# actuday6418/ray-tracer-s8

Hardware: AMD Instinct MI355X
Metric: Mrays/sec @ 4K/8spp 1024-sphere (higher is better)
Workload: dtype f32

## Files before the change

### ray_tracer_s8_amd/csrc/rt_api.hip

```cpp
#include <hip/hip_runtime.h>
#include <dlfcn.h>

#include <algorithm>
#include <chrono>
#include <cmath>
#include <cstdarg>
#include <cstdio>
#include <cstdlib>
#include <cstring>
#include <atomic>
#include <climits>
#include <condition_variable>
#include <memory>
#include <mutex>
#include <new>
#include <stdexcept>
#include <string>
#include <thread>
#include <vector>

#include "rt_assign.h"
#include "rt_bvh.h"
#include "rt_device.h"
#include "rt_frame_plan.h"
#include "rt_kernel.hip.h"
#include "rt_plan.h"
#include "rt_query.hip.h"
#include "rt_scene_host.h"
#include "rt_trace.hip.h"
#include "rt_bounce.hip.h"
#include "rt_direct.hip.h"
#include "rt_nee.hip.h"
#include "rt_aov.hip.h"
#include "rt_camera.hip.h"
#include "rt_denoise.hip.h"
#include "rt_tile.h"
#ifdef RT_DEBUG_HOOKS
#include "rt_unit.hip.h"
#endif

namespace {

thread_local std::string g_err;

int fail(int code, const std::string& msg) {
    g_err = msg;
    return code;
}

void set_err_noexcept(const char* what) noexcept {
    try {
        g_err = what;
    } catch (...) {
    }
}
template <class F>
int guarded(F&& body) noexcept {
    try {
        return body();
    } catch (const std::bad_alloc&) {
        set_err_noexcept("host allocation failed");
        return RT_ERR_OOM;
    } catch (const std::exception& e) {
        set_err_noexcept(e.what());
        return RT_ERR_HIP;
    } catch (...) {
        set_err_noexcept("internal error");
        return RT_ERR_HIP;
    }
}

#define HIPCHK(expr)                                                                                  \
    do {                                                                                              \
        hipError_t _e = (expr);                                                                       \
        if (_e != hipSuccess)                                                                         \
            return fail(RT_ERR_HIP, std::string(#expr) + ": " + hipGetErrorString(_e) + " (" __FILE__ \
                                                                                        ":" +         \
                                        std::to_string(__LINE__) + ")");                              \
    } while (0)

using rtdev::DevArray;
using rtdev::Event;
using rtdev::EventPool;
using rtdev::GrowBuf;
using rtdev::Stream;

int reserve(GrowBuf& buf, size_t bytes, const char* what) {
    if (buf.grow(bytes) == hipSuccess) return RT_OK;
    (void)hipGetLastError();
    return fail(RT_ERR_OOM, std::string("hipMalloc(") + what + ") failed");
}

struct DeviceCtx {
    int dev = -1;
    Stream stream;
    Stream copy_stream;
    int n_cu = 0;
    std::mutex mu;
};

enum DebugKnob {
    DBG_LDS_TREE = 0,
    DBG_CULL_WALK,
    DBG_NO_STAGE,
    DBG_SLOTS,
    DBG_FORCE_CAPPED,
    DBG_STACK_LDS,
    DBG_COMPACT,
    DBG_REFILL_EIGHTHS,
    DBG_COMMIT_SLOTS,
    DBG_VERBOSE,
    DBG_REORDER,
    DBG_TAIL_TILES,
    DBG_STRIP_COST,
    DBG_DENOISE_LDS_STEP,
    DBG_N
};
std::atomic<int> g_dbg[DBG_N];
const struct { const char* env; int def; } g_dbg_spec[DBG_N] = {
    {"RT_LDS_TREE", 1}, {"RT_CULL_WALK", -1}, {"RT_NO_STAGE", 0}, {"RT_SLOTS", 0}, {"RT_FORCE_CAPPED", 0},
    {"RT_STACK_LDS", 0}, {"RT_COMPACT", 1}, {"RT_REFILL_EIGHTHS", 0}, {"RT_COMMIT_SLOTS", 0}, {"RT_VERBOSE", 0}, {"RT_REORDER", 1}, {"RT_TAIL_TILES", -1}, {"RT_STRIP_COST", 1},
    {"RT_DENOISE_LDS_STEP", -1}};
std::once_flag g_dbg_once;
void dbg_load_env() {
    std::call_once(g_dbg_once, [] {
        for (int k = 0; k < DBG_N; k++) {
            const char* e = getenv(g_dbg_spec[k].env);
            int v = g_dbg_spec[k].def;
            if (e) v = k == DBG_VERBOSE ? 1 : atoi(e);
            g_dbg[k].store(v, std::memory_order_relaxed);
        }
    });
}
inline int dbg(DebugKnob k) { return g_dbg[k].load(std::memory_order_relaxed); }

std::mutex g_mu;
bool g_init = false;
std::vector<DeviceCtx*> g_ctx;
std::atomic<int> g_live_scenes{0};

rtplan::Knobs plan_knobs() {
    rtplan::Knobs k;
    k.lds_tree = dbg(DBG_LDS_TREE);
    k.cull_walk = dbg(DBG_CULL_WALK);
    k.no_stage = dbg(DBG_NO_STAGE);
    k.slots = dbg(DBG_SLOTS);
    k.commit_slots = dbg(DBG_COMMIT_SLOTS);
    k.force_capped = dbg(DBG_FORCE_CAPPED);
    k.stack_lds = dbg(DBG_STACK_LDS);
    k.compact = dbg(DBG_COMPACT);
    k.refill_eighths = dbg(DBG_REFILL_EIGHTHS);
    k.tail_tiles = dbg(DBG_TAIL_TILES);
    return k;
}

}

struct rt_scene {
    DeviceCtx* ctx = nullptr;
    rtplan::SceneShape shape;
    uint32_t n_lights = 0;
    DevArray<uint32_t> d_lights;
    DevArray<float> d_light_c;
    DevArray<float> d_light_ip;
    float light_total = 0.f;
    std::vector<uint32_t> light_world;
    std::vector<float> light_p;
    rtplan::Pose pose;
    bool has_pose = false;
    uint32_t light_sampling = RT_LIGHTS_AREA;
    uint32_t glossy_sampling = RT_GLOSSY_BOUNCE;
    DevArray<float4> d_geom;
    DevArray<float4> d_geom_pk;
    DevArray<float4> d_geom_px;
    DevArray<float4> d_mat;
    DevArray<float> d_emis;
    DevArray<float> d_tri;
    DevArray<float4> d_tri_box;
    DevArray<float4> d_bvh;
    DevArray<float4> d_trav;
    GrowBuf stack_ovf;
    DevArray<uint4> d_travq;
    DevArray<float4> d_geom_r;
    DevArray<uint32_t> d_big;
    uint32_t n_big = 0;
    float tri_k = 0.f, tri_diag = 0.f, tri_es = 0.f, tri_e = 0.f;
    rtbvh::QGrid grid;
    DevArray<uint32_t> d_leaf_of;
    DevArray<uint32_t> d_world_rank;
    bool has_order = false;
    float bvh_build_ms = 0.f;
    DevArray<unsigned long long> d_counters;
    struct Ring {
        GrowBuf buf;
        hipStream_t last = nullptr;
        uint64_t stamp = 0;
    };
    Ring rings[4];
    uint64_t ring_clock = 0;
    GrowBuf d_out, d_outf, d_acc, d_cost;
    GrowBuf d_stage;
    EventPool events;
    uint64_t primary_rays = 0;
    float h2d_ms = 0.f;
    uint32_t last_engine = 0, last_form = 0;
    std::mutex mu;
};

namespace {

int check_request(const rt_tile_request* rq) {
    if (!rq) return fail(RT_ERR_BAD_ARG, "request is NULL");
    if (rq->width == 0 || rq->height == 0 || rq->divisions == 0 || rq->spp == 0)
        return fail(RT_ERR_BAD_ARG, "width, height, divisions and spp must be non-zero");
    if (rq->division_no >= rq->divisions) return fail(RT_ERR_BAD_ARG, "division_no >= divisions");
    if (rq->height / rq->divisions == 0) return fail(RT_ERR_BAD_ARG, "height / divisions == 0 rows");
    if (rq->max_bounces > RT_MAX_BOUNCES) return fail(RT_ERR_LIMIT, "max_bounces > RT_MAX_BOUNCES");
    if (rq->spp > RT_MAX_SPP) return fail(RT_ERR_LIMIT, "spp > RT_MAX_SPP");
    if (rq->reserved != 0) return fail(RT_ERR_BAD_ARG, "reserved must be 0");
    if ((uint64_t)rq->width * rq->height > 0x7fffffffull) return fail(RT_ERR_LIMIT, "image too large");
    return RT_OK;
}

constexpr uint32_t QUEUE_SLOTS = 16384;
#ifdef RT_PROFILE_TIME
constexpr uint32_t COUNTER_WORDS = 4 + QUEUE_SLOTS + 16 * 8192;
#else
constexpr uint32_t COUNTER_WORDS = 4 + QUEUE_SLOTS;
#endif

int check_slot(const rt_scene* sc) {
    if (sc->events.pending().size() >= QUEUE_SLOTS) return fail(RT_ERR_LIMIT, "too many uncollected launches: call rt_scene_collect()");
    return RT_OK;
}

template <class P>
int enqueue(rt_scene* sc, hipStream_t stream, void (*kern)(const P), uint32_t blocks, uint32_t block, size_t lds, const P& p) {
    EventPool::Lease ev;
    int rc = check_slot(sc);
    if (rc) return rc;
    HIPCHK(sc->events.lease(ev));
    HIPCHK(hipEventRecord(ev.a(), stream));
    hipLaunchKernelGGL(kern, dim3(blocks), dim3(block), lds, stream, p);
    HIPCHK(hipGetLastError());
    HIPCHK(hipEventRecord(ev.b(), stream));
    ev.to_pending();
    return RT_OK;
}

struct Grid {
    uint32_t blocks = 0;
    int per_cu = 0;
};
template <class P>
int persistent_blocks(const rt_scene* sc, void (*kern)(const P), uint32_t block, size_t lds, uint64_t items, Grid& g) {
    HIPCHK(hipOccupancyMaxActiveBlocksPerMultiprocessor(&g.per_cu, kern, (int)block, lds));
    if (g.per_cu < 1) g.per_cu = 1;
    g.blocks = (uint32_t)std::min<uint64_t>((items + block - 1) / block, (uint64_t)sc->ctx->n_cu * (uint32_t)g.per_cu);
    return RT_OK;
}

void scene_refs(const rt_scene* sc, bool full_chain, rtk::SceneRefs& r) {
    r.n_sph = sc->shape.n_sph;
    r.n_tri = sc->shape.n_tri;
    r.root_ref = sc->shape.root_ref;
    r.full_chain = full_chain ? 1u : 0u;
    r.trav = sc->d_trav.get();
    r.bvh_nodes = sc->d_bvh.get();
    r.leaf_of = sc->d_leaf_of.get();
    r.world_rank = sc->has_order ? sc->d_world_rank.get() : nullptr;
    r.geom_r = sc->d_geom_r.get();
    r.tri = sc->d_tri.get();
    r.counters = sc->d_counters.get();
}

struct Pass {
    uint32_t begin, end;
    void* const* d_acc;
};
int acquire_stack_ovf(rt_scene* sc, size_t words) {
    HIPCHK(sc->stack_ovf.grow(words * sizeof(uint32_t)));
    return RT_OK;
}

int acquire_ring(rt_scene* sc, hipStream_t stream, size_t bytes, rt_scene::Ring*& rg) {
    rg = nullptr;
    for (auto& r : sc->rings)
        if (r.buf.data() && r.last == stream) { rg = &r; break; }
    if (!rg)
        for (auto& r : sc->rings)
            if (!r.buf.data()) { rg = &r; break; }
    if (!rg) {
        rg = &sc->rings[0];
        for (auto& r : sc->rings)
            if (r.stamp < rg->stamp) rg = &r;
    }
    HIPCHK(rg->buf.grow(bytes));
    if (!rg->buf.done) HIPCHK(rg->buf.done.create(hipEventDisableTiming));
    else if (rg->last != stream) HIPCHK(hipStreamWaitEvent(stream, rg->buf.done.get(), 0));
    rg->last = stream;
    rg->stamp = ++sc->ring_clock;
    return RT_OK;
}

int launch_batch(rt_scene* sc, const rt_tile_request* rqs, uint32_t n, void* const* d_rgb, void* const* d_f32,
                 hipStream_t stream, unsigned long long* d_strip_cost = nullptr, const Pass* pass = nullptr) {
    const rtplan::Knobs kn = plan_knobs();
    const rtplan::SceneShape& sh = sc->shape;
    rtk::KParams p;
    std::memset(&p, 0, sizeof p);
    const rtplan::SampleRange smp = pass ? rtplan::SampleRange{pass->begin, pass->end, true} : rtplan::SampleRange{0u, rqs[0].spp, false};
    rtplan::Plan pl = rtplan::plan_launch(sh, rqs[0], n, smp, kn, p, sc->has_pose ? &sc->pose : nullptr);
    if (pl.status != RT_OK) return fail(pl.status, pl.error);
    p.geom_pk = sc->d_geom_pk.get();
    p.geom_px = sc->d_geom_px.get();
    p.geom = sc->d_geom.get();
    p.mat = sc->d_mat.get();
    p.emis = sc->d_emis.get();
    p.tri = sc->d_tri.get();
    p.tri_box = sc->d_tri_box.get();
    p.bvh_nodes = sc->d_bvh.get();
    p.trav = sc->d_trav.get();
    p.travq = sc->d_travq.get();
    p.geom_r = sc->d_geom_r.get();
    for (int i = 0; i < 3; i++) {
        p.q_base[i] = sc->grid.base[i];
        p.q_step[i] = sc->grid.step[i];
        p.q_rstep[i] = 1.0f / sc->grid.step[i];
    }
    p.leaf_of = sc->d_leaf_of.get();
    p.world_rank = sc->has_order ? sc->d_world_rank.get() : nullptr;
    p.big = sc->d_big.get();
    p.n_big = sc->n_big;
    p.r_slack = sh.r_slack;
    p.tri_k = sc->tri_k;
    p.tri_diag = sc->tri_diag;
    p.tri_es = sc->tri_es;
    p.tri_e = sc->tri_e;
    for (uint32_t i = 0; i < n; i++) {
        p.strips[i].seed = rqs[i].seed;
        p.strips[i].rgb = (uint8_t*)d_rgb[i];
        p.strips[i].f32 = d_f32 ? (float*)d_f32[i] : nullptr;
        p.strips[i].acc = pass ? (float*)pass->d_acc[i] : nullptr;
        p.strips[i].y0 = p.Hs * rqs[i].division_no;
    }
    int rc = check_slot(sc);
    if (rc) return rc;
    p.counters = sc->d_counters.get();
    p.queue = sc->d_counters.get() + 4 + sc->events.pending().size();
    p.strip_cost = dbg(DBG_STRIP_COST) ? d_strip_cost : nullptr;

    const rtk::KernelFn kern = pl.isect < 2 ? rtk::kernel_linear(pl.isect, pl.expanded) : rtk::kernel_traverse(pl.isect, pl.count_steps);
    int per_cu = 0;
    HIPCHK(hipOccupancyMaxActiveBlocksPerMultiprocessor(&per_cu, kern, pl.block, pl.lds));
    if (per_cu < 1) per_cu = 1;
    if (dbg(DBG_VERBOSE))
        fprintf(stderr, "[rt] engine %d%s  lds %zu B  workgroups/CU %d  leaf slots %u  bvh depth %u  leaf density %.3f  prims %u\n",
                pl.engine, pl.capped ? " (capped stack)" : "", pl.lds, per_cu, pl.maxl_l2, sh.bvh_depth, sh.leaf_density, sh.n_sph + sh.n_tri);
    rtplan::plan_queue(pl, (uint32_t)sc->ctx->n_cu * (uint32_t)per_cu, kn, p);
    p.stack_ovf = nullptr;
    if (pl.capped) {
        if ((rc = acquire_stack_ovf(sc, pl.ovf_words))) return rc;
        p.stack_ovf = (uint32_t*)sc->stack_ovf.data();
    }
    if (dbg(DBG_VERBOSE))
        fprintf(stderr, "[rt] sample-unit ring %zu B: %u units per pixel, %u slots of %u records per wave\n", pl.ring_bytes, p.upp, p.n_slots,
                p.slot_stride);
    rt_scene::Ring* rg = nullptr;
    if ((rc = acquire_ring(sc, stream, pl.ring_bytes, rg))) return rc;
    p.ring = (float*)rg->buf.data();
    if (p.stack_ovf) {
        if (sc->stack_ovf.done) HIPCHK(hipStreamWaitEvent(stream, sc->stack_ovf.done.get(), 0));
        else HIPCHK(sc->stack_ovf.done.create(hipEventDisableTiming));
    }
    HIPCHK(hipMemsetAsync(p.queue, 0, sizeof(unsigned long long), stream));
    sc->last_engine = (uint32_t)pl.engine;
    sc->last_form = pl.expanded ? 1u : 0u;
    if ((rc = enqueue(sc, stream, kern, pl.blocks, pl.block, pl.lds, p))) return rc;
    HIPCHK(hipEventRecord(rg->buf.done.get(), stream));
    if (p.stack_ovf) HIPCHK(hipEventRecord(sc->stack_ovf.done.get(), stream));
    sc->primary_rays += (uint64_t)p.Hs * p.W * p.upp * n;
    return RT_OK;
}

int collect_locked(rt_scene* sc, rt_tile_stats* st) {
    float ms = 0.f;
    uint32_t n = 0;
    for (const EventPool::Pair& pr : sc->events.pending()) {
        HIPCHK(hipEventSynchronize(pr.b));
        float t = 0.f;
        HIPCHK(hipEventElapsedTime(&t, pr.a, pr.b));
        ms += t;
        n++;
    }
    sc->events.collected();
    unsigned long long c[4] = {0, 0, 0, 0};
    HIPCHK(hipMemcpy(c, sc->d_counters.get(), sizeof c, hipMemcpyDeviceToHost));
    HIPCHK(hipMemset(sc->d_counters.get(), 0, sizeof c));
    if (st) {
        st->ray_segments = c[0];
        st->broad_candidates = c[1];
        st->exact_fallbacks = c[2];
        st->primary_rays = sc->primary_rays;
        st->kernel_ms = ms;
        st->n_launches = n;
        st->h2d_ms = sc->h2d_ms;
        st->d2h_ms = 0.f;
        st->engine = sc->last_engine;
        st->broad_form = sc->last_form;
        st->node_steps = c[3];
    }
    sc->primary_rays = 0;
    sc->h2d_ms = 0.f;
    return RT_OK;
}

struct StagedCall {
    rt_scene* const sc;
    const hipStream_t st;
    const float scene_h2d_ms;
    EventPool::Lease up, down;
    bool finished = false;
    explicit StagedCall(rt_scene* s) : sc(s), st(s->ctx->stream.get()), scene_h2d_ms(s->h2d_ms) {}
    StagedCall(const StagedCall&) = delete;
    ~StagedCall() {
        if (!finished) (void)hipStreamSynchronize(st);
        sc->h2d_ms = scene_h2d_ms;
    }
    int begin() {
        int rc = collect_locked(sc, nullptr);
        if (rc) return rc;
        HIPCHK(sc->events.lease(up));
        HIPCHK(sc->events.lease(down));
        HIPCHK(hipEventRecord(up.a(), st));
        return RT_OK;
    }
    int uploads_done() {
        HIPCHK(hipEventRecord(up.b(), st));
        return RT_OK;
    }
    int kernels_done() {
        HIPCHK(hipEventRecord(down.a(), st));
        return RT_OK;
    }
    int finish(rt_tile_stats* stats) {
        HIPCHK(hipEventRecord(down.b(), st));
        HIPCHK(hipEventSynchronize(down.b()));
        finished = true;
        rt_tile_stats s;
        float h2d = 0.f, d2h = 0.f;
        HIPCHK(hipEventElapsedTime(&h2d, up.a(), up.b()));
        HIPCHK(hipEventElapsedTime(&d2h, down.a(), down.b()));
        int rc = collect_locked(sc, &s);
        if (rc) return rc;
        s.h2d_ms = h2d;
        s.d2h_ms = d2h;
        if (stats) *stats = s;
        return RT_OK;
    }
};

__attribute__((format(printf, 1, 2))) std::string vtext(const char* fmt, ...) {
    if (!dbg(DBG_VERBOSE)) return {};
    char buf[256];
    va_list ap;
    va_start(ap, fmt);
    vsnprintf(buf, sizeof buf, fmt, ap);
    va_end(ap);
    return buf;
}

template <class P>
void material_refs(const rt_scene* sc, P& p) {
    p.mat = sc->d_mat.get();
    p.emis = sc->d_emis.get();
}
template <class P>
void light_refs(const rt_scene* sc, P& p) {
    p.lights = sc->d_lights.get();
    p.n_lights = sc->n_lights;
    p.table.light_c = sc->d_light_c.get();
    p.table.light_ip = sc->d_light_ip.get();
    p.table.light_total = sc->light_total;
}

static bool lights_by_power(uint32_t flags) { return (flags & RT_FLAG_LIGHTS_BY_POWER) != 0; }
static bool lights_cone(const rt_scene* sc) { return sc->light_sampling == RT_LIGHTS_CONE; }
static bool glossy_mis(const rt_scene* sc, const rt_nee_request* rq) { return sc->glossy_sampling == RT_GLOSSY_MIS && rq->mode == RT_NEE_MIS; }

template <class P>
int launch_persistent(rt_scene* sc, int engine, size_t lds, uint32_t block, void (*kern)(const P), const char* what, const P& p,
                      uint64_t items, const std::string& head, const std::string& tail, uint64_t primary, hipStream_t stream,
                      void* d_zero = nullptr) {
    if (!kern) return fail(RT_ERR_HIP, std::string("no ") + what + " kernel for this plan");
    Grid g;
    int rc = persistent_blocks(sc, kern, block, lds, items, g);
    if (rc || (d_zero && (rc = check_slot(sc)))) return rc;
    if (dbg(DBG_VERBOSE)) fprintf(stderr, "[rt] %sworkgroups/CU %d  %s\n", head.c_str(), g.per_cu, tail.c_str());
    if (d_zero) HIPCHK(hipMemsetAsync(d_zero, 0, sizeof(uint32_t), stream));
    if ((rc = enqueue(sc, stream, kern, g.blocks, block, lds, p))) return rc;
    sc->primary_rays += primary;
    sc->last_engine = (uint32_t)engine;
    sc->last_form = 0;
    return RT_OK;
}

template <class P>
int launch_rays(rt_scene* sc, const rtplan::QueryPlan& qp, uint32_t block, void (*kern)(const P), const char* what, P& p, uint64_t items,
                const std::string& head, const std::string& tail, uint64_t primary, hipStream_t stream, void* d_zero = nullptr) {
    scene_refs(sc, qp.full_chain, p);
    return launch_persistent(sc, qp.engine, qp.lds, block, kern, what, p, items, head, tail, primary, stream, d_zero);
}

template <class P>
void frame_refs(const rt_scene* sc, const rt_tile_request& rq, uint32_t begin, P& p) {
    rtplan::fill_camera(rq, sc->has_pose ? &sc->pose : nullptr, p);
    p.t_min = rq.t_min;
    p.t_max = rq.t_max;
    p.W = rq.width;
    p.H = rq.height;
    p.spp_all = rq.spp;
    p.s_begin = begin;
}

template <class L>
int device_form(rt_scene* sc, void* hip_stream, L&& launch) {
    std::lock_guard<std::mutex> lk(sc->mu);
    HIPCHK(hipSetDevice(sc->ctx->dev));
    return launch(hip_stream ? (hipStream_t)hip_stream : sc->ctx->stream.get());
}

struct HostForm {
    rt_scene* const sc;
    std::lock_guard<std::mutex> dl, lk;
    explicit HostForm(rt_scene* s) : sc(s), dl(s->ctx->mu), lk(s->mu) {}
    int device() const {
        HIPCHK(hipSetDevice(sc->ctx->dev));
        return RT_OK;
    }
};

struct Staging {
    enum : unsigned { UP = rtplan::STAGE_UP, DOWN = rtplan::STAGE_DOWN, DEVICE = rtplan::STAGE_DEVICE };
    using Entry = rtplan::StageEntry;
    GrowBuf& buf;
    std::vector<Entry> e;
    const size_t total;
    Staging(rt_scene* sc, std::vector<Entry> entries) : buf(sc->d_stage), e(std::move(entries)), total(rtplan::stage_layout(e.data(), e.size())) {}
    int reserve(const char* what) { return ::reserve(buf, total, what); }
    char* dev(size_t k) const { return e[k].present() ? buf.data() + e[k].off : nullptr; }
    int upload(StagedCall& call) const {
        for (int k = 0; k < (int)e.size(); k++)
            if (e[k].host && e[k].bytes && (e[k].copy & UP)) HIPCHK(hipMemcpyAsync(dev(k), e[k].host, e[k].bytes, hipMemcpyHostToDevice, call.st));
        return call.uploads_done();
    }
    int download(StagedCall& call) const {
        int rc = call.kernels_done();
        if (rc) return rc;
        for (int k = 0; k < (int)e.size(); k++)
            if (e[k].host && e[k].bytes && (e[k].copy & DOWN))
                HIPCHK(hipMemcpyAsync(const_cast<void*>(e[k].host), dev(k), e[k].bytes, hipMemcpyDeviceToHost, call.st));
        return RT_OK;
    }
};

int check_active_list(const uint32_t* active, uint32_t n_active, uint32_t n) {
    if (!active) return RT_OK;
    if (n_active > n) return fail(RT_ERR_BAD_ARG, "n_active > n");
    for (uint32_t k = 0; k < n_active; k++)
        if (active[k] >= n) return fail(RT_ERR_BAD_ARG, "active[" + std::to_string(k) + "] >= n");
    return RT_OK;
}

}

extern "C" {

RT_API uint32_t rt_abi_version(void) { return RT_ABI_VERSION; }

RT_API const char* rt_strerror(int status) {
    switch (status) {
        case RT_OK: return "ok";
        case RT_ERR_BAD_ARG: return "bad argument";
        case RT_ERR_NOT_INITIALIZED: return "rt_init() has not succeeded";
        case RT_ERR_NO_DEVICE: return "no HIP device (this library has no CPU fallback)";
        case RT_ERR_BAD_DEVICE: return "device ordinal out of range";
        case RT_ERR_BUFFER_TOO_SMALL: return "output buffer smaller than (height/divisions)*width*3";
        case RT_ERR_FRAME_SIZE: return "height is not a multiple of divisions";
        case RT_ERR_HIP: return "HIP runtime error";
        case RT_ERR_LIMIT: return "limit exceeded";
        case RT_ERR_OOM: return "out of memory";
        default: return "unknown status";
    }
}

RT_API const char* rt_last_error(void) { return g_err.c_str(); }

RT_API void rt_tile_request_defaults(rt_tile_request* rq) {
    if (!rq) return;
    std::memset(rq, 0, sizeof *rq);
    rq->width = 1920;
    rq->height = 1080;
    rq->divisions = 20;
    rq->division_no = 0;
    rq->spp = 100;
    rq->max_bounces = 10;
    rq->aperture = 0.1f;
    rq->focus_distance = 1.0f;
    rq->fov = 3.14159265358979323846f / 2.0f;
    rq->focal_length = 1.0f;
    rq->t_min = 0.001f;
    rq->t_max = 1000.0f;
    rq->seed = 0;
    rq->flags = RT_FLAG_NONE;
}

RT_API size_t rt_tile_bytes(const rt_tile_request* rq) {
    return rq ? rtframe::strip_bytes(*rq) : 0;
}

static int rt_init_impl(int* n_devices) {
    dbg_load_env();
    std::lock_guard<std::mutex> lk(g_mu);
    if (g_init) {
        if (n_devices) *n_devices = (int)g_ctx.size();
        return RT_OK;
    }
    int n = 0;
    hipError_t e = hipGetDeviceCount(&n);
    if (e != hipSuccess || n <= 0) {
        if (n_devices) *n_devices = 0;
        return fail(RT_ERR_NO_DEVICE, std::string("hipGetDeviceCount: ") +
                                          (e != hipSuccess ? hipGetErrorString(e) : "0 devices"));
    }
    for (int d = 0; d < n; d++) {
        DeviceCtx* c = new DeviceCtx;
        c->dev = d;
        g_ctx.push_back(c);
    }
    g_init = true;
    if (n_devices) *n_devices = n;
    return RT_OK;
}

static int ensure_ctx(DeviceCtx* c) {
    std::lock_guard<std::mutex> lk(c->mu);
    if (c->stream) return RT_OK;
    HIPCHK(hipSetDevice(c->dev));
    HIPCHK(hipDeviceGetAttribute(&c->n_cu, hipDeviceAttributeMultiprocessorCount, c->dev));
    for (int isect = 0; isect < rtplan::N_ISECT; isect++)
        for (int alt = 0; alt < 2; alt++)
            HIPCHK(hipFuncSetAttribute((const void*)(isect < 2 ? rtk::kernel_linear(isect, alt != 0) : rtk::kernel_traverse(isect, alt != 0)),
                                       hipFuncAttributeMaxDynamicSharedMemorySize, (int)rtplan::LDS_LIMIT));
    Stream st, cs;
    HIPCHK(st.create(hipStreamNonBlocking));
    HIPCHK(cs.create(hipStreamNonBlocking));
    c->copy_stream = std::move(cs);
    c->stream = std::move(st);
    return RT_OK;
}

static int rt_shutdown_impl(void) {
    std::lock_guard<std::mutex> lk(g_mu);
    if (g_live_scenes.load() > 0)
        return fail(RT_ERR_BAD_ARG, "rt_shutdown() refused: destroy every rt_scene first (their device contexts stay valid)");
    for (DeviceCtx* c : g_ctx) {
        (void)hipSetDevice(c->dev);
        delete c;
    }
    g_ctx.clear();
    g_init = false;
    return RT_OK;
}

static int rt_scene_destroy_impl(rt_scene* sc);

using rtscene::HostScene;
static_assert(sizeof(rtscene::F4) == sizeof(float4) && alignof(rtscene::F4) == alignof(float4), "HostScene's records are the device's float4");

static int check_world(const rt_sphere* sp, uint32_t ns, const rt_triangle* tr, uint32_t nt, const uint32_t* world_index) {
    if ((ns && !sp) || (nt && !tr)) return fail(RT_ERR_BAD_ARG, "primitive pointer is NULL");
    if ((uint64_t)ns + nt > RT_MAX_PRIMITIVES) return fail(RT_ERR_LIMIT, "too many primitives (RT_MAX_PRIMITIVES)");
    if (world_index && !rtscene::world_is_permutation(world_index, ns + nt))
        return fail(RT_ERR_BAD_ARG, "world_index is not a permutation of 0 .. n_spheres + n_triangles - 1");
    return RT_OK;
}

static int upload_scene(int device, const HostScene& hs, rt_scene** out) {
    const auto t_create0 = std::chrono::steady_clock::now();
    if (!g_init) return fail(RT_ERR_NOT_INITIALIZED, "call rt_init() first");
    if (device < 0 || device >= (int)g_ctx.size()) return fail(RT_ERR_BAD_DEVICE, "bad device ordinal");
    DeviceCtx* ctx = g_ctx[device];
    {
        int rc0 = ensure_ctx(ctx);
        if (rc0) return rc0;
    }
    HIPCHK(hipSetDevice(ctx->dev));
    struct Destroy {
        void operator()(rt_scene* s) const { rt_scene_destroy_impl(s); }
    };
    std::unique_ptr<rt_scene, Destroy> sc(new (std::nothrow) rt_scene);
    if (!sc) return fail(RT_ERR_OOM, "host allocation failed");
    g_live_scenes.fetch_add(1);
    const rtbvh::FlatBVH& bvh = hs.bvh;
    sc->ctx = ctx;
    sc->shape = hs.shape;
    sc->bvh_build_ms = hs.bvh_build_ms;
    sc->grid = bvh.grid;
    sc->has_order = hs.has_order;
    sc->n_lights = hs.n_lights;
    sc->light_total = hs.light_total;
    sc->light_p.assign(hs.light_p.begin(), hs.light_p.begin() + hs.n_lights);
    sc->light_world.resize(hs.n_lights);
    for (uint32_t k = 0; k < hs.n_lights; k++) sc->light_world[k] = hs.has_order ? hs.world_rank[hs.lights[k]] : hs.lights[k];
    sc->n_big = hs.n_big;
    sc->tri_k = hs.tri_k;
    sc->tri_diag = hs.tri_diag;
    sc->tri_es = hs.tri_es;
    sc->tri_e = hs.tri_e;
    const hipStream_t st = ctx->stream.get();
    Event e0, e1;
    if (e0.create() != hipSuccess || e1.create() != hipSuccess) return fail(RT_ERR_HIP, "hipEventCreate failed");
    int rc = RT_OK;
    auto step = [&](hipError_t e, const char* what) {
        if (e != hipSuccess) rc = fail(e == hipErrorOutOfMemory ? RT_ERR_OOM : RT_ERR_HIP, std::string("scene upload, ") + what + ": " + hipGetErrorString(e));
    };
    auto up = [&](auto& dst, const auto& vec, const char* what) {
        if (!rc) step(dst.upload(vec, st), what);
    };
    step(hipEventRecord(e0.get(), st), "hipEventRecord");
    up(sc->d_geom, hs.geom, "geom");
    up(sc->d_geom_pk, hs.geom_pk, "geom_pk");
    up(sc->d_geom_px, hs.geom_px, "geom_px");
    up(sc->d_mat, hs.mat, "mat");
    up(sc->d_emis, hs.emis, "emis");
    up(sc->d_tri, hs.tri, "tri");
    up(sc->d_tri_box, hs.tri_box, "tri_box");
    up(sc->d_bvh, bvh.nodes, "bvh nodes");
    up(sc->d_leaf_of, bvh.leaf_of, "leaf_of");
    up(sc->d_world_rank, hs.world_rank, "world_rank");
    up(sc->d_trav, bvh.trav, "trav");
    up(sc->d_travq, bvh.travq, "travq");
    up(sc->d_geom_r, hs.geom_r, "geom_r");
    up(sc->d_big, hs.big, "big");
    up(sc->d_lights, hs.lights, "lights");
    up(sc->d_light_c, hs.light_c, "light_c");
    up(sc->d_light_ip, hs.light_ip_prim, "light_ip");
    if (!rc) step(sc->d_counters.alloc(COUNTER_WORDS), "counters");
    if (!rc) step(hipMemsetAsync(sc->d_counters.get(), 0, COUNTER_WORDS * sizeof(unsigned long long), st), "hipMemsetAsync(counters)");
    if (!rc) step(hipEventRecord(e1.get(), st), "hipEventRecord");
    if (!rc) step(hipEventSynchronize(e1.get()), "hipEventSynchronize");
    if (!rc) step(hipEventElapsedTime(&sc->h2d_ms, e0.get(), e1.get()), "hipEventElapsedTime");
    if (rc) return rc;
    if (dbg(DBG_VERBOSE))
        fprintf(stderr, "[rt] scene: %u prims  culled walk: %u big spheres, slack radius %g, box density %.3f -> %s  bvh build %.2f ms (host)  uploads %.2f ms  upload total %.2f ms\n",
                hs.shape.n_sph + hs.shape.n_tri, hs.n_big, hs.shape.r_slack, hs.shape.cull_density, hs.shape.cull_pays ? "default" : "off", sc->bvh_build_ms, sc->h2d_ms,
                std::chrono::duration<float, std::milli>(std::chrono::steady_clock::now() - t_create0).count());
    *out = sc.release();
    return RT_OK;
}

static int rt_scene_create_impl(int device, const rt_sphere* sp, uint32_t ns, const rt_triangle* tr, uint32_t nt,
                                const uint32_t* world_index, rt_scene** out) {
    if (!out) return fail(RT_ERR_BAD_ARG, "out_scene is NULL");
    *out = nullptr;
    int rc = check_world(sp, ns, tr, nt, world_index);
    if (rc) return rc;
    if (!g_init) return fail(RT_ERR_NOT_INITIALIZED, "call rt_init() first");
    if (device < 0 || device >= (int)g_ctx.size()) return fail(RT_ERR_BAD_DEVICE, "bad device ordinal");
    HostScene hs;
    rtscene::build_host_scene(sp, ns, tr, nt, world_index, dbg(DBG_REORDER) != 0, hs);
    return upload_scene(device, hs, out);
}

static int rt_scene_destroy_impl(rt_scene* sc) {
    if (!sc) return RT_OK;
    if (sc->ctx) (void)hipSetDevice(sc->ctx->dev);
    for (const EventPool::Pair& pr : sc->events.pending()) (void)hipEventSynchronize(pr.b);
    delete sc;
    g_live_scenes.fetch_sub(1);
    return RT_OK;
}

static int check_batch(const rt_tile_request* rqs, uint32_t n) {
    if (!rqs || n == 0) return fail(RT_ERR_BAD_ARG, "empty request batch");
    for (uint32_t i = 0; i < n; i++) {
        int rc = check_request(&rqs[i]);
        if (rc) return rc;
        if (!rtframe::same_frame(rqs[0], rqs[i]))
            return fail(RT_ERR_BAD_ARG, "batched requests must agree on every field but division_no and seed");
    }
    return RT_OK;
}

static int check_samples(uint32_t begin, uint32_t end, uint32_t spp) {
    if (begin >= end) return fail(RT_ERR_BAD_ARG, "sample_begin >= sample_end");
    if (end > spp) return fail(RT_ERR_BAD_ARG, "sample_end > spp");
    return RT_OK;
}

static int check_array(const void* const* a, uint32_t n, const char* what) {
    if (!a) return fail(RT_ERR_BAD_ARG, std::string(what) + " is NULL");
    for (uint32_t i = 0; i < n; i++)
        if (!a[i]) return fail(RT_ERR_BAD_ARG, std::string(what) + "[i] is NULL");
    return RT_OK;
}
// ... 756 lines not shown
            sd.f32 = f32 ? (float*)f32[b0 + i] : nullptr;
            sd.lin = lin ? (float*)lin[b0 + i] : nullptr;
        }
    };
    auto grid_stride = [&](uint64_t pixels) { return (uint32_t)std::min<uint64_t>((pixels + 255) / 256, persist); };
    auto tiles = [&](uint32_t rows) { return pl.tiles_x * ((rows + rtplan::DN_TILE_Y - 1) / rtplan::DN_TILE_Y); };
    int rc;
    p.dst = buf[0];
    for (uint32_t b0 = 0; b0 < n; b0 += rtk::DN_BAND) {
        band(b0, std::min<uint32_t>(rtk::DN_BAND, n - b0));
        if ((rc = launch(rtk::dn_entry_kernel(), grid_stride((uint64_t)p.rows * W), 0))) return rc;
    }
    uint32_t cur = 0;
    float kc = dq.k_color;
    for (uint32_t i = 0; i < dq.iterations; i++) {
        p.s = pl.step[i];
        p.kc = kc;
        p.src = buf[cur];
        p.dst = buf[cur ^ 1u];
        const bool last = i + 1 == dq.iterations;
        const rtk::DnFn kern = rtk::dn_step_kernel(pl.lds[i] != 0, last);
        if (!last) {
            p.row0 = 0;
            p.rows = R;
            p.n_strips = 0;
            if ((rc = launch(kern, tiles(R), pl.lds[i]))) return rc;
        } else {
            for (uint32_t b0 = 0; b0 < n; b0 += rtk::DN_BAND) {
                band(b0, std::min<uint32_t>(rtk::DN_BAND, n - b0));
                if ((rc = launch(kern, tiles(p.rows), pl.lds[i]))) return rc;
            }
        }
        if (dbg(DBG_VERBOSE))
            fprintf(stderr, "[rt] denoise: iteration %u  step %u  lds %zu B  workgroups/CU %u  image %u x %u  planes %#x\n", i, p.s,
                    pl.lds[i], pl.wg_per_cu[i], W, R, mask);
        cur ^= 1u;
        kc = kc * dq.color_step_scale;
    }
    if (dq.iterations == 0) {
        p.src = buf[0];
        for (uint32_t b0 = 0; b0 < n; b0 += rtk::DN_BAND) {
            band(b0, std::min<uint32_t>(rtk::DN_BAND, n - b0));
            if ((rc = launch(rtk::dn_output_kernel(), grid_stride((uint64_t)p.rows * W), 0))) return rc;
        }
    }
    sc->last_engine = 0;
    sc->last_form = 0;
    return RT_OK;
}

static int rt_scene_denoise_device_impl(rt_scene* sc, const rt_tile_request* rqs, uint32_t n, const rt_denoise_request* dq,
                                        const void* const* d_acc, const rt_aov_planes* d_planes, void* const* d_rgb, size_t out_len,
                                        void* const* d_f32, void* const* d_lin, void* d_scratch, size_t scratch_bytes,
                                        void* hip_stream) {
    uint32_t mask = 0;
    int rc = check_denoise(sc, rqs, n, dq, d_acc, d_planes, (const void* const*)d_rgb, out_len, (const void* const*)d_f32,
                           (const void* const*)d_lin, &mask);
    if (rc) return rc;
    const uint32_t R = rqs[0].height / rqs[0].divisions * n;
    if (!d_scratch) return fail(RT_ERR_BAD_ARG, "d_scratch is NULL");
    if (scratch_bytes < rtplan::plan_denoise(rqs[0].width, R, 0, false).scratch_bytes)
        return fail(RT_ERR_BAD_ARG, "scratch_bytes < rt_denoise_scratch_bytes(W, R)");
    return device_form(sc, hip_stream, [&](hipStream_t st) {
        return launch_denoise(sc, rqs, n, *dq, mask, d_acc, d_planes, d_rgb, d_f32, d_lin, (char*)d_scratch, st);
    });
}

static int rt_scene_denoise_impl(rt_scene* sc, const rt_tile_request* rqs, uint32_t n, const rt_denoise_request* dq,
                                 const float* const* acc, const rt_aov_planes* planes, uint8_t* const* rgb, size_t out_len,
                                 float* const* f32, float* const* lin, rt_tile_stats* stats) {
    uint32_t mask = 0;
    int rc = check_denoise(sc, rqs, n, dq, (const void* const*)acc, planes, (const void* const*)rgb, out_len,
                           (const void* const*)f32, (const void* const*)lin, &mask);
    if (rc) return rc;
    HostForm hf(sc);
    Staging s(sc, rtplan::dn_stage_list(rqs[0], n, acc, planes, rgb, f32, lin));
    StagedCall call(sc);
    auto launch = [&] {
        std::vector<const void*> d_acc(n);
        std::vector<rt_aov_planes> d_pl(n);
        std::vector<void*> d_rgb(n), d_f32(n), d_lin(n);
        for (uint32_t i = 0; i < n; i++) {
            auto dev = [&](int k) { return s.dev(1 + (size_t)rtplan::DN_STAGE_STRIP * i + k); };
            d_acc[i] = dev(rtplan::DN_ACCUM);
            d_pl[i] = {(float*)dev(rtplan::DN_ALBEDO), (float*)dev(rtplan::DN_NORMAL), (float*)dev(rtplan::DN_DEPTH),
                       (uint32_t*)dev(rtplan::DN_HITS), nullptr};
            d_rgb[i] = dev(rtplan::DN_RGB);
            d_f32[i] = dev(rtplan::DN_F32);
            d_lin[i] = dev(rtplan::DN_LIN);
        }
        return launch_denoise(sc, rqs, n, *dq, mask, d_acc.data(), d_pl.data(), rgb ? d_rgb.data() : nullptr, f32 ? d_f32.data() : nullptr,
                              lin ? d_lin.data() : nullptr, s.dev(0), call.st);
    };
    if ((rc = hf.device()) || (rc = s.reserve("denoise staging")) || (rc = call.begin()) || (rc = s.upload(call)) || (rc = launch()) ||
        (rc = s.download(call)))
        return rc;
    return call.finish(stats);
}

#ifdef RT_DEBUG_HOOKS
extern "C" __attribute__((visibility("default"))) int rt_debug_read_counters(rt_scene* sc, uint32_t first, uint32_t n,
                                                                             unsigned long long* out) {
    return guarded([&]() -> int {
        if (!sc || !out || first > COUNTER_WORDS || n > COUNTER_WORDS - first) return fail(RT_ERR_BAD_ARG, "counter range");
        std::lock_guard<std::mutex> lk(sc->mu);
        HIPCHK(hipSetDevice(sc->ctx->dev));
        HIPCHK(hipMemcpy(out, sc->d_counters.get() + first, n * sizeof(unsigned long long), hipMemcpyDeviceToHost));
        return RT_OK;
    });
}
extern "C" __attribute__((visibility("default"))) int rt_debug_sqrt_selftest(int device, uint32_t from, unsigned long long n,
                                                                             unsigned long long* mismatches) {
    return guarded([&]() -> int {
        if (!mismatches || n > (1ull << 32) - from) return fail(RT_ERR_BAD_ARG, "sqrt self-test range");
        HIPCHK(hipSetDevice(device));
        DevArray<unsigned long long> d_bad;
        HIPCHK(d_bad.alloc(1));
        hipError_t e = hipMemset(d_bad.get(), 0, sizeof(unsigned long long));
        if (e == hipSuccess) {
            rtk::sqrt_selftest_launch(from, n, d_bad.get(), 0);
            e = hipGetLastError();
        }
        if (e == hipSuccess) e = hipMemcpy(mismatches, d_bad.get(), sizeof(unsigned long long), hipMemcpyDeviceToHost);
        if (e != hipSuccess) return fail(RT_ERR_HIP, hipGetErrorString(e));
        return RT_OK;
    });
}
extern "C" __attribute__((visibility("default"))) int rt_debug_unit(int device, int unit, int family, unsigned long long n,
                                                                    const void* in, void* out) {
    return guarded([&]() -> int {
        if (!rtk::unit_instantiated(unit, family)) return fail(RT_ERR_BAD_ARG, "unit / family");
        if (n == 0) return RT_OK;
        if (!in || !out || n > (1ull << 24)) return fail(RT_ERR_BAD_ARG, "unit records");
        const size_t bi = (size_t)n * rtk::unit_record_in(family) * 4, bo = (size_t)n * rtk::unit_record_out(family) * 4;
        HIPCHK(hipSetDevice(device));
        DevArray<uint32_t> d_in, d_out;
        hipError_t e = d_in.alloc(bi / 4);
        if (e == hipSuccess) e = d_out.alloc(bo / 4);
        if (e == hipSuccess) e = hipMemcpy(d_in.get(), in, bi, hipMemcpyHostToDevice);
        if (e == hipSuccess) e = hipMemset(d_out.get(), 0, bo);
        if (e == hipSuccess) {
            rtk::unit_launch(unit, family, n, d_in.get(), d_out.get(), 0);
            e = hipGetLastError();
        }
        if (e == hipSuccess) e = hipDeviceSynchronize();
        if (e == hipSuccess) e = hipMemcpy(out, d_out.get(), bo, hipMemcpyDeviceToHost);
        if (e != hipSuccess) return fail(RT_ERR_HIP, hipGetErrorString(e));
        return RT_OK;
    });
}
extern "C" __attribute__((visibility("default"))) int rt_debug_set(const char* name, int value) {
    dbg_load_env();
    if (!name) return INT32_MIN;
    for (int k = 0; k < DBG_N; k++)
        if (!strcmp(name, g_dbg_spec[k].env)) return g_dbg[k].exchange(value);
    return INT32_MIN;
}
extern "C" __attribute__((visibility("default"))) int rt_debug_throw(int kind) {
    return guarded([&]() -> int {
        if (kind == 0) throw std::bad_alloc();
        if (kind == 1) throw std::runtime_error("rt_debug_throw");
        if (kind == 2) throw 42;
        if (kind == 3) { std::vector<char> v; v.reserve((size_t)-1 / 2); }
        return RT_OK;
    });
}
#endif

static int rt_render_tile_impl(int device, const rt_tile_request* rq, const rt_sphere* sp, uint32_t ns,
                          const rt_triangle* tr, uint32_t nt, const uint32_t* world_index, uint8_t* out_rgb, size_t out_len,
                          float* out_f32, rt_tile_stats* stats) {
    int rc = check_request(rq);
    if (rc) return rc;
    if (!out_rgb) return fail(RT_ERR_BAD_ARG, "out_rgb is NULL");
    if (out_len < rt_tile_bytes(rq)) return fail(RT_ERR_BUFFER_TOO_SMALL, "out_len < (H/div)*W*3");
    rt_scene* sc = nullptr;
    rc = rt_scene_create_impl(device, sp, ns, tr, nt, world_index, &sc);
    if (rc) return rc;
    rc = rt_scene_render_tile_impl(sc, rq, out_rgb, out_len, out_f32, stats);
    std::string keep = g_err;
    rt_scene_destroy_impl(sc);
    if (rc) g_err = keep;
    return rc;
}

}

struct FrameDev {
    int dev = 0;
    rt_scene* scene = nullptr;
    std::thread th;
    Stream qs[2];
    GrowBuf qd[2];
    int rc = RT_OK;
    std::string err;
    rt_tile_stats st;
    float busy_ms = 0.f;
};

struct rt_frame_ctx {
    std::vector<FrameDev> fd;
    std::mutex call_mu;
    std::mutex mu;
    std::condition_variable cv_work, cv_done;
    uint64_t gen = 0;
    int pending = 0;
    enum Cmd { CMD_NONE, CMD_UPLOAD, CMD_RENDER, CMD_STOP } cmd = CMD_NONE;
    const HostScene* hs = nullptr;
    bool have_world = false;
    float scene_ms_pending = 0.f;
    rtplan::Pose pose;
    bool has_pose = false;
    rtframe::CostMemory costs;
    void* pinned_ptr = nullptr;
    size_t pinned_len = 0;
    rtframe::FramePlan plan;
    uint8_t* out = nullptr;
    std::atomic<uint32_t> next_strip{0};
    std::vector<unsigned long long> cost_now;
};

namespace {

int frame_dev_render_owned(rt_frame_ctx* fc, int w) {
    FrameDev& d = fc->fd[w];
    const rtframe::FramePlan& plan = fc->plan;
    std::vector<rt_tile_request> rqs;
    std::vector<uint8_t*> outs;
    for (uint32_t k = 0; k < plan.rq.divisions; k++) {
        if (plan.owner[k] != (uint32_t)w) continue;
        rt_tile_request rq = plan.rq;
        rq.division_no = k;
        rqs.push_back(rq);
        outs.push_back(fc->out + (size_t)k * plan.strip_bytes);
    }
    if (rqs.empty()) return RT_OK;
    std::vector<unsigned long long> cost(rqs.size(), 0ull);
    int r = rt_scene_render_tiles_impl(d.scene, rqs.data(), (uint32_t)rqs.size(), outs.data(), plan.strip_bytes, nullptr, &d.st, cost.data());
    if (r) return r;
    for (size_t i = 0; i < rqs.size(); i++) fc->cost_now[rqs[i].division_no] = cost[i];
    return RT_OK;
}

int frame_dev_render_queue(rt_frame_ctx* fc, int w) {
    FrameDev& d = fc->fd[w];
    const rt_tile_request& rq0 = fc->plan.rq;
    const size_t strip = fc->plan.strip_bytes;
    uint8_t* out_rgb = fc->out;
    rt_scene* sc = d.scene;
    HIPCHK(hipSetDevice(sc->ctx->dev));
    for (int i = 0; i < 2; i++)
        if (!d.qs[i]) HIPCHK(d.qs[i].create(hipStreamNonBlocking));
    for (int i = 0; i < 2; i++) {
        int rc = reserve(d.qd[i], strip, "strip");
        if (rc) return rc;
    }
    bool busy[2] = {false, false};
    struct Settle {
        FrameDev& d;
        bool* busy;
        ~Settle() {
            for (int i = 0; i < 2; i++)
                if (busy[i]) (void)hipStreamSynchronize(d.qs[i].get());
        }
    } settle{d, busy};
    for (uint32_t turn = 0;; turn++) {
        const int sl = (int)(turn & 1u);
        if (busy[sl]) {
            HIPCHK(hipStreamSynchronize(d.qs[sl].get()));
            busy[sl] = false;
        }
        const uint32_t i = fc->next_strip.fetch_add(1);
        if (i >= rq0.divisions) break;
        rt_tile_request rq = rq0;
        rq.division_no = rq0.divisions - 1u - i;
        void* d1[1] = {d.qd[sl].data()};
        int r = rt_scene_render_tiles_device_impl(sc, &rq, 1, d1, strip, nullptr, d.qs[sl].get());
        if (r) return r;
        HIPCHK(hipMemcpyAsync(out_rgb + (size_t)rq.division_no * strip, d.qd[sl].data(), strip, hipMemcpyDeviceToHost, d.qs[sl].get()));
        busy[sl] = true;
    }
    for (int i = 0; i < 2; i++)
        if (busy[i]) {
            HIPCHK(hipStreamSynchronize(d.qs[i].get()));
            busy[i] = false;
        }
    return rt_scene_collect_impl(sc, &d.st);
}

int frame_dev_render(rt_frame_ctx* fc, int w) {
    FrameDev& d = fc->fd[w];
    std::memset(&d.st, 0, sizeof d.st);
    rt_scene* sc = d.scene;
    if (!sc) return fail(RT_ERR_BAD_ARG, "rt_frame_ctx_render before rt_frame_ctx_set_world");
    {
        std::lock_guard<std::mutex> lk(sc->mu);
        sc->pose = fc->pose;
        sc->has_pose = fc->has_pose;
    }
    return fc->plan.mode == rtassign::QUEUE ? frame_dev_render_queue(fc, w) : frame_dev_render_owned(fc, w);
}

void frame_dev_release(FrameDev& d) {
    rt_scene_destroy_impl(d.scene);
    d.scene = nullptr;
    (void)hipSetDevice(d.dev);
// ... 443 lines not shown
```

### ray_tracer_s8_amd/csrc/rt_kernel.hip.h

```cpp
#pragma once
#include <hip/hip_runtime.h>
#include <type_traits>
#include <stdint.h>

#include "rt_consts.h"
#include "rt_cull.h"

namespace rtk {

#ifndef RT_MINWAVES
#define RT_MINWAVES 4
#endif
#ifndef RT_MINWAVES_TRAV
#define RT_MINWAVES_TRAV 4
#endif
#ifndef RT_MINWAVES_LTREE
#define RT_MINWAVES_LTREE 4
#endif
#ifndef RT_MINWAVES_CULL
#define RT_MINWAVES_CULL 5
#endif
#ifndef RT_STEPS_PER_CHECK_X
#define RT_STEPS_PER_CHECK_X 16
#endif
#ifndef RT_QUEUE_TAKE_MIN
#define RT_QUEUE_TAKE_MIN 4
#endif
#ifndef RT_BF2
#define RT_BF2 1
#endif
#ifndef RT_CULL_FLUSH_MIN
#define RT_CULL_FLUSH_MIN 1
#endif
#ifndef RT_MINWAVES_QTRAV
#define RT_MINWAVES_QTRAV 5
#endif
#ifndef RT_STEPS_PER_CHECK
#define RT_STEPS_PER_CHECK 8
#endif
#ifndef RT_STEPS_PER_CHECK_LTREE
#define RT_STEPS_PER_CHECK_LTREE 8
#endif
#ifndef RT_STEPS_PER_CHECK_Q
#define RT_STEPS_PER_CHECK_Q 16
#endif
#ifndef RT_LT_PARTIAL
#define RT_LT_PARTIAL 40
#endif
#ifndef RT_LT_EAGER
#define RT_LT_EAGER 12
#endif

constexpr uint32_t SLOT_FREE = 0x80000000u;
struct WaveQ {
    uint32_t cnt[SLOTS_MAX];
    uint32_t cost_acc[2];
    uint32_t cost_strip[2];
};
static_assert(sizeof(WaveQ) == 144, "WaveQ layout (rt_plan.h: LDS_LIMIT leaves 3 KiB of static LDS)");
constexpr uint32_t SLOT_UNIT_BITS = 13;
struct WaveStage {
    int left[STAGE_TILES + 1];
    uint32_t dst_lo[STAGE_TILES + 1], dst_hi[STAGE_TILES + 1];
};

struct StripDesc {
    uint64_t seed;
    uint8_t* rgb;
    float* f32;
    float* acc;
    uint32_t y0;
    uint32_t pad;
};

struct KParams {
    uint32_t W, H, Hs;
    uint32_t upp, depth;
    uint32_t spp_all, s_begin, gap;
    uint32_t acc_out;
    uint32_t n_sph, n_sph_pad;
    uint32_t n_tri;
    uint32_t chunk;
    uint32_t n_chunks;
    uint32_t flags;
    uint32_t path32;
    uint32_t lds_cand_off;
    uint32_t lds_path_off;
    uint32_t lds_rr_off;
    uint32_t lds_stack_off;
    uint32_t lds_cmp_off;
    uint32_t lds_stage_off;
    uint32_t n_strips;
    uint32_t tiles_x, tiles_per_strip;
    uint32_t tiles_total;
    uint32_t tiles_big;
    uint32_t sub_shift;
    uint32_t n_tiles;
    uint32_t n_slots;
    uint32_t grp;
    uint32_t grp_magic;
    uint32_t slot_stride;
    uint32_t commit_slots;
    uint32_t spp_magic;
    uint32_t slotu_magic;
    float* ring;
    float org[3], llc[3], hor[3], ver[3];
    float lens_radius, focus_distance;
    float lens_u[3], lens_v[3];
    float u_den, v_den;
    float t_min, t_max;
    float spp_f;
    float spp_rcp;
    const float4* geom_pk;
    const float4* geom_px;
    const float4* geom;
    const float4* mat;
    const float* emis;
    const float* tri;
    const float4* tri_box;
    const float4* trav;
    const uint4* travq;
    const float4* geom_r;
    float q_base[3], q_step[3], q_rstep[3];
    uint32_t root_ref;
    uint32_t maxl;
    uint32_t list16;
    uint32_t stack_lds;
    uint32_t ovf_stride;
    uint32_t* stack_ovf;
    const uint32_t* big;
    uint32_t n_big;
    float r_slack;
    float tri_k, tri_diag, tri_es, tri_e;
    uint32_t refill_eighths;
    uint32_t n_internal;
    uint32_t lds_node_off;
    const float4* bvh_nodes;
    const uint32_t* leaf_of;
    const uint32_t* world_rank;
    unsigned long long* strip_cost;
    unsigned long long* counters;
    unsigned long long* queue;
    StripDesc strips[MAX_BATCH];
};

struct V3 {
    float x, y, z;
};
__device__ __forceinline__ V3 mk(float x, float y, float z) { return V3{x, y, z}; }
__device__ __forceinline__ V3 operator+(V3 a, V3 b) { return {a.x + b.x, a.y + b.y, a.z + b.z}; }
__device__ __forceinline__ V3 operator-(V3 a, V3 b) { return {a.x - b.x, a.y - b.y, a.z - b.z}; }
__device__ __forceinline__ V3 operator*(float s, V3 a) { return {s * a.x, s * a.y, s * a.z}; }
__device__ __forceinline__ V3 operator*(V3 a, float s) { return {a.x * s, a.y * s, a.z * s}; }
template <class P>
__device__ __forceinline__ V3 lens_offset(const P& p, float x1, float x2) {
    return mk(x1 * p.lens_u[0] + x2 * p.lens_v[0], x1 * p.lens_u[1] + x2 * p.lens_v[1], x1 * p.lens_u[2] + x2 * p.lens_v[2]);
}
template <bool NEG_OK = false>
__device__ __forceinline__ float sqrt_rn(float x) {
#ifdef RT_IEEE_SQRT_PLAIN
    return __builtin_sqrtf(x);
#else
    const float r = __builtin_amdgcn_rsqf(x);
    float g = x * r, h = 0.5f * r;
    const float e = __builtin_fmaf(-h, g, 0.5f);
    g = __builtin_fmaf(g, e, g);
    h = __builtin_fmaf(h, e, h);
    const float dd = __builtin_fmaf(-g, g, x);
    float y = __builtin_fmaf(dd, h, g);
    const bool odd = ((__float_as_uint(x) & (NEG_OK ? 0x7fffffffu : 0xffffffffu)) - 0x0f800000u) >= (0x7f800000u - 0x0f800000u);
    if (__ballot(odd)) {
        if (odd) {
            asm volatile("" : "+v"(x));
            y = __builtin_sqrtf(x);
        }
    }
    return y;
#endif
}
#define RT_SQRT(x_) sqrt_rn(x_)
#define RT_SQRT_NEG_OK(x_) sqrt_rn<true>(x_)
#define RT_DIV(a_, b_) ((a_) / (b_))
#define RT_HOOK_LT_STEP_LOADS(nd_, ni_, lnodes_)
#define RT_HOOK_LT_STEP_ALU(p0_, p1_, p2_, p3_, oy_)
#define RT_HOOK_LT_STEP_END
#define RT_HOOK_Q_GATHER(t_ref_, cl_, travq_, n_internal_)
#ifdef RT_PROBES
#include "rt_probes.h"
#endif
__device__ __forceinline__ V3 operator/(V3 a, float s) { return {RT_DIV(a.x, s), RT_DIV(a.y, s), RT_DIV(a.z, s)}; }
__device__ __forceinline__ float dot(V3 a, V3 b) { return (a.x * b.x + a.y * b.y) + a.z * b.z; }
__device__ __forceinline__ float vlength(V3 a) { return RT_SQRT(dot(a, a)); }
__device__ __forceinline__ V3 normalize(V3 a) { return a / vlength(a); }
__device__ __forceinline__ bool try_normalize(V3 a, V3& out) {
    float rcp = RT_DIV(1.0f, RT_SQRT(dot(a, a)));
    if (rcp > 0.0f && rcp < __builtin_inff()) {
        out = a * rcp;
        return true;
    }
    return false;
}
__device__ __forceinline__ V3 normalize_or_zero(V3 a) {
    V3 r;
    return try_normalize(a, r) ? r : mk(0.f, 0.f, 0.f);
}
__device__ __forceinline__ V3 cross(V3 a, V3 b) {
    return {a.y * b.z - a.z * b.y, a.z * b.x - a.x * b.z, a.x * b.y - a.y * b.x};
}

struct Rng {
    uint64_t s0, s1, s2, s3;
};
__device__ __forceinline__ uint64_t rotl64(uint64_t x, int k) { return (x << k) | (x >> (64 - k)); }
__device__ __forceinline__ uint32_t next_u32(Rng& r) {
    uint64_t result = rotl64(r.s0 + r.s3, 23) + r.s0;
    uint64_t t = r.s1 << 17;
    r.s2 ^= r.s0;
    r.s3 ^= r.s1;
    r.s1 ^= r.s2;
    r.s0 ^= r.s3;
    r.s2 ^= t;
    r.s3 = rotl64(r.s3, 45);
    return (uint32_t)(result >> 32);
}
__device__ __forceinline__ uint64_t splitmix_mix(uint64_t z) {
    z = (z ^ (z >> 30)) * 0xbf58476d1ce4e5b9ull;
    z = (z ^ (z >> 27)) * 0x94d049bb133111ebull;
    return z ^ (z >> 31);
}
constexpr uint64_t PHI = 0x9e3779b97f4a7c15ull;
__device__ __forceinline__ Rng seed_state(uint64_t st) {
    Rng r;
    st += PHI; r.s0 = splitmix_mix(st);
    st += PHI; r.s1 = splitmix_mix(st);
    st += PHI; r.s2 = splitmix_mix(st);
    st += PHI; r.s3 = splitmix_mix(st);
    return r;
}
__device__ __forceinline__ float u01(Rng& r) {
    return __uint_as_float((next_u32(r) >> 9) | 0x3f800000u) - 1.0f;
}
__device__ __forceinline__ float gen_range_01(Rng& r) { return u01(r) * 1.0f + 0.0f; }
__device__ __forceinline__ float uniform_m1_1(Rng& r) { return u01(r) * 2.0f + -1.0f; }

__device__ __forceinline__ bool exact_sphere(V3 o, V3 td, V3 cen, float rr, float t_min, float t_max,
                                             float& t_out) {
    const V3 oc = o - cen;
    const float b = dot(td, oc);
    const float len = RT_SQRT(dot(oc, oc));
    const float c = len * len - rr;
    const float disc = b * b - 4.0f * c;
    const float sq = RT_SQRT_NEG_OK(disc);
    const bool bneg = b < 0.0f;
    const float same_sign = bneg ? -b + sq : -b - sq;
    const float diff_sign = bneg ? -b - sq : -b + sq;
    const float a0x2 = 2.0f * c;
    const bool big_s = __builtin_fabsf(same_sign) > 2.0f, big_d = __builtin_fabsf(diff_sign) > 2.0f;
    const float q1 = RT_DIV(a0x2, same_sign), q2 = RT_DIV(a0x2, diff_sign), hs = same_sign / 2.0f, hd = diff_sign / 2.0f;
    const float x1 = big_s ? q1 : hd;
    const float x2 = big_s ? (big_d ? q2 : hs) : hs;
    const bool one = disc == 0.0f;
    const float r1 = -b / 2.0f;
    const float x = one ? r1 : (x1 < x2 ? x1 : x2);
    const float y = one ? r1 : (x1 < x2 ? x2 : x1);
    const bool xin = (x >= t_min) && (x < t_max);
    const bool yin = (y >= t_min) && (y < t_max);
    t_out = (xin && yin) ? (x < y ? x : y) : (xin ? x : y);
    return !(disc < 0.0f) && (xin || yin);
}

__device__ __forceinline__ bool exact_triangle(V3 o, V3 d, const float* __restrict__ tv, float t_min, float t_max,
                                               float& t_out) {
    const float EPSILON = 0.00001f;
    V3 A = mk(tv[0], tv[1], tv[2]), B = mk(tv[3], tv[4], tv[5]), C = mk(tv[6], tv[7], tv[8]);
    V3 a_to_b = B - A;
    V3 a_to_c = C - A;
    V3 u_vec = cross(d, a_to_c);
    float det = dot(a_to_b, u_vec);
    if (det < EPSILON && det > -EPSILON) return false;
    float inv_det = 1.0f / det;
    V3 a_to_origin = o - A;
    float u = dot(a_to_origin, u_vec) * inv_det;
    if (!(u >= 0.0f && u <= 1.0f)) return false;
    V3 v_vec = cross(a_to_origin, a_to_b);
    float v = dot(d, v_vec) * inv_det;
    if (v < 0.0f || u + v > 1.0f) return false;
    float dist = dot(a_to_c, v_vec) * inv_det;
    if (!(dist > EPSILON)) return false;
    t_out = dist;
    return (dist >= t_min) && (dist < t_max);
}

struct RayAux {
    V3 inv;
    bool sx, sy, sz;
    bool full_chain;
// ... 48 lines not shown
    for (;;) {
        const float4 lo = nodes[2 * (size_t)node];
        const uint32_t parent = __float_as_uint(lo.w);
        if (parent == 0xffffffffu) return true;
        const float4 hi = nodes[2 * (size_t)node + 1];
        if (!intersects_aabb(o, a, lo, hi)) return false;
        if (finite_inv) return true;
        node = parent;
    }
}

struct Hit {
    int idx;
    float dist;
    float t;
};
template <int MODE>
__device__ __forceinline__ void consider(Hit& h, int idx, V3 o, V3 d, float t, const RayAux& a,
                                         const float4* __restrict__ nodes, const uint32_t* __restrict__ leaf_of) {
    V3 p = o + t * d;
    float dist = vlength(p - o);
    const bool better = h.idx < 0 || h.dist > dist;
    const bool tie = h.idx >= 0 && h.dist == dist;
    if (!(better || tie)) return;
    if (MODE == 0) {
        if (!better) return;
    } else if (MODE == 1) {
        if (!better && leaf_of[idx] > leaf_of[h.idx]) return;
    } else {
        const uint32_t rank = leaf_of[idx];
        if (!better && rank > leaf_of[h.idx]) return;
        if (!bvh_reaches(nodes, rank, o, a)) return;
    }
    h.idx = idx;
    h.dist = dist;
    h.t = t;
}

template <bool RANKED = false, class Pred>
__device__ __forceinline__ void consider_if(Hit& h, int idx, V3 o, V3 d, float t, Pred admitted, const uint32_t* __restrict__ leaf_of = nullptr) {
    V3 p = o + t * d;
    float dist = vlength(p - o);
    if (!(h.idx < 0 || h.dist > dist)) {
        if (!(RANKED && h.dist == dist && leaf_of[idx] < leaf_of[h.idx])) return;
    }
    if (!admitted()) return;
    h.idx = idx;
    h.dist = dist;
    h.t = t;
}

__device__ __forceinline__ unsigned long long wave_sum(unsigned long long v) {
    for (int off = 32; off > 0; off >>= 1) v += __shfl_xor(v, off, 64);
    return v;
}

__device__ __forceinline__ uint8_t f32_as_u8(float v) {
    if (!(v == v)) return 0;
    if (v <= 0.0f) return 0;
    if (v >= 255.0f) return 255;
    return (uint8_t)(int)v;
}

#ifdef RT_PROFILE_PHASES
#define WCOUNT(slot)                                                                         \
    do {                                                                                     \
        unsigned long long _m = __ballot(1);                                                 \
        if ((int)(threadIdx.x & 63) == (int)__builtin_ctzll(_m)) atomicAdd(&p.counters[4 + 8192 + (slot)], 1ull); \
    } while (0)
#define LCOUNT(slot)                                                                         \
    do {                                                                                     \
        unsigned long long _m = __ballot(1);                                                 \
        if ((int)(threadIdx.x & 63) == (int)__builtin_ctzll(_m)) {                           \
            atomicAdd(&p.counters[4 + 8192 + 32 + (slot)], (unsigned long long)__builtin_popcountll(_m)); \
            atomicAdd(&p.counters[4 + 8192 + 64 + (slot)], 1ull);                            \
        }                                                                                    \
    } while (0)
#else
#define WCOUNT(slot) do { } while (0)
#define LCOUNT(slot) do { } while (0)
#endif
#ifdef RT_PROFILE_TIME
#define TDECL unsigned long long _tacc[8] = {0, 0, 0, 0, 0, 0, 0, 0}; unsigned long long _tlast = __builtin_amdgcn_s_memtime(); const unsigned long long _t0 = __builtin_amdgcn_s_memrealtime(); unsigned long long _tq = 0, _nq = 0
#define TDRAINED do { _tq = __builtin_amdgcn_s_memrealtime(); } while (0)
#define TROUND do { if (_tq) { const uint32_t _w = blockIdx.x * (blockDim.x >> 6) + (threadIdx.x >> 6); const unsigned long long _lv = __builtin_popcountll(__ballot(have_unit)); \
    if ((threadIdx.x & 63) == 0 && _w % 20u == 0u && _w / 20u < 215u && _nq < 16ull) p.counters[4 + 8192 + 4400 + (_w / 20u) * 16u + _nq] = (__builtin_amdgcn_s_memrealtime() & 0xfffffffull) | (_lv << 28); \
    _nq++; } } while (0)
#define TSTAMP(ph) do { const unsigned long long _n = __builtin_amdgcn_s_memtime(); _tacc[ph] += _n - _tlast; _tlast = _n; } while (0)
#define TFLUSH do { if ((threadIdx.x & 63) == 0) { const uint32_t _w = blockIdx.x * (blockDim.x >> 6) + (threadIdx.x >> 6); \
    if (_w < 8192u) { unsigned long long* _b = p.counters + 4 + 16384 + 16u * _w; for (int _i = 0; _i < 8; _i++) _b[_i] = _tacc[_i]; \
    _b[8] = __builtin_amdgcn_s_memrealtime(); _b[9] = _t0; _b[10] = _tq; _b[11] = _nq; } } } while (0)
#else
#define TDECL do { } while (0)
#define TDRAINED do { } while (0)
#define TROUND do { } while (0)
#define TSTAMP(ph) do { } while (0)
#define TFLUSH do { } while (0)
#endif

#ifndef RT_GEOM_RR
#define RT_SPHERE_REC(p_, prim_) ([&]() { const float4 r_ = at32((p_).geom_r, (prim_)); return make_float4(r_.x, r_.y, r_.z, r_.w * r_.w); }())
#else
#define RT_SPHERE_REC(p_, prim_) at32((p_).geom, (prim_))
#endif

typedef float v2f __attribute__((ext_vector_type(2)));
__device__ __forceinline__ v2f pk_fma(v2f a, v2f b, v2f c) { return __builtin_elementwise_fma(a, b, c); }

template <class T>
__device__ __forceinline__ const T& at32(const T* __restrict__ base, uint32_t i) {
    return *reinterpret_cast<const T*>(reinterpret_cast<const char*>(base) + i * (uint32_t)sizeof(T));
}

template <bool ON>
__device__ __forceinline__ int cold(int v) {
    if (ON) asm volatile("" : "+v"(v));
    return v;
}
#ifndef RT_COMMIT_BATCH
#define RT_COMMIT_BATCH 8
#endif
#ifndef RT_COMMIT_AGENT_LOADS
#define RT_COMMIT_AGENT_LOADS 0
#endif
template <class T>
__device__ __forceinline__ T ring_load(const T* q) {
#if RT_COMMIT_AGENT_LOADS
    return __hip_atomic_load(q, __ATOMIC_RELAXED, __HIP_MEMORY_SCOPE_AGENT);
#else
    return *q;
#endif
}
__device__ __forceinline__ uint32_t uni(uint32_t v) { return (uint32_t)__builtin_amdgcn_readfirstlane((int)v); }

__device__ __forceinline__ void qslabs(const uint4 qa, const uint4 qb, V3 ig, V3 cq, float& lmin, float& lmax, float& rmin_, float& rmax_) {
#define RT_Q(word, hi16) ((float)((hi16) ? ((word) >> 16) : ((word) & 0xffffu)))
    const float ax = __builtin_fabsf(ig.x), ay = __builtin_fabsf(ig.y), az = __builtin_fabsf(ig.z);
    const float lcx = __builtin_fmaf(RT_Q(qa.x, 0), ig.x, cq.x), lcy = __builtin_fmaf(RT_Q(qa.x, 1), ig.y, cq.y), lcz = __builtin_fmaf(RT_Q(qa.y, 0), ig.z, cq.z);
    const float lhx = RT_Q(qa.y, 1), lhy = RT_Q(qa.z, 0), lhz = RT_Q(qa.z, 1);
    const float rcx = __builtin_fmaf(RT_Q(qa.w, 0), ig.x, cq.x), rcy = __builtin_fmaf(RT_Q(qa.w, 1), ig.y, cq.y), rcz = __builtin_fmaf(RT_Q(qb.x, 0), ig.z, cq.z);
    const float rhx = RT_Q(qb.x, 1), rhy = RT_Q(qb.y, 0), rhz = RT_Q(qb.y, 1);
#undef RT_Q
    lmin = __builtin_fmaxf(__builtin_fmaxf(__builtin_fmaf(-lhx, ax, lcx), __builtin_fmaf(-lhy, ay, lcy)), __builtin_fmaf(-lhz, az, lcz));
    lmax = __builtin_fminf(__builtin_fminf(__builtin_fmaf(lhx, ax, lcx), __builtin_fmaf(lhy, ay, lcy)), __builtin_fmaf(lhz, az, lcz));
    rmin_ = __builtin_fmaxf(__builtin_fmaxf(__builtin_fmaf(-rhx, ax, rcx), __builtin_fmaf(-rhy, ay, rcy)), __builtin_fmaf(-rhz, az, rcz));
    rmax_ = __builtin_fminf(__builtin_fminf(__builtin_fmaf(rhx, ax, rcx), __builtin_fmaf(rhy, ay, rcy)), __builtin_fmaf(rhz, az, rcz));
}

__device__ __forceinline__ float cull_bound(float best, V3 o, float r_slack) { return cull_bound(best, o.x, o.y, o.z, r_slack); }
__device__ __forceinline__ float cull_bound_tri(float best, V3 o, float k, float diag, float es, float e) {
    return cull_bound_tri(best, o.x, o.y, o.z, k, diag, es, e);
}

template <int ISECT, bool EXPANDED, int BS = BLOCK, bool STATS = false>
__global__ __launch_bounds__(BS, (ISECT == 5 || ISECT == 6) ? RT_MINWAVES_LTREE : ISECT == 9 ? RT_MINWAVES_TRAV : ISECT >= 7 ? RT_MINWAVES_CULL : ISECT >= 3 ? RT_MINWAVES_QTRAV : ISECT == 2 ? RT_MINWAVES_TRAV : RT_MINWAVES) void rt_tile_kernel(const KParams p) {
    constexpr int BLOCK = BS;
    constexpr bool STREAMED = (ISECT == 1);
    constexpr bool TRAVERSE = (ISECT >= 2);
    constexpr bool QNODES = (ISECT == 3 || ISECT == 4 || ISECT == 7 || ISECT == 8);
    constexpr bool CULL = (ISECT == 6 || ISECT == 7 || ISECT == 8 || ISECT == 9);
    constexpr bool XNODES = (ISECT == 2 || ISECT == 9);
    constexpr bool CAPPED = (ISECT == 4 || ISECT == 8);
    constexpr bool LTREE = (ISECT == 5 || ISECT == 6);
    constexpr uint32_t LB = LTREE ? 0x8000u : LEAF_BIT;
    constexpr bool BFSTEP = LTREE;
    const uint32_t ML = QNODES ? p.maxl : (uint32_t)MAXL_EXACT;
    extern __shared__ __attribute__((aligned(16))) unsigned char lds_raw[];
    __shared__ unsigned long long wg_tiles;
    __shared__ unsigned int wg_lock, wg_drained;
    __shared__ WaveQ wave_q[BS / 64];
    constexpr bool CAN_STAGE = (ISECT >= 1 && ISECT <= 4) || ISECT >= 7;
    __shared__ WaveStage wave_st[CAN_STAGE ? BS / 64 : 1];
    {
        uint32_t* z = reinterpret_cast<uint32_t*>(&wave_q[threadIdx.x >> 6]);
        if ((threadIdx.x & 63u) < SLOTS_MAX) wave_q[threadIdx.x >> 6].cnt[threadIdx.x & 63u] = SLOT_FREE;
        if ((threadIdx.x & 63u) == 0u) {
            wave_q[threadIdx.x >> 6].cost_acc[0] = wave_q[threadIdx.x >> 6].cost_acc[1] = 0u;
            wave_q[threadIdx.x >> 6].cost_strip[0] = wave_q[threadIdx.x >> 6].cost_strip[1] = 0xffffffffu;
        }
        (void)z;
        if (CAN_STAGE && (threadIdx.x & 63u) <= STAGE_TILES) wave_st[threadIdx.x >> 6].left[threadIdx.x & 63u] = -1;
    }
    if (threadIdx.x == 0) {
        wg_tiles = 0ull;
        wg_lock = 0u;
        wg_drained = 0u;
    }
    __syncthreads();
    float4* lgeom = reinterpret_cast<float4*>(lds_raw);
    const float* lgeomf = reinterpret_cast<const float*>(lds_raw);
    float* lrr = reinterpret_cast<float*>(lds_raw + p.lds_rr_off);
    const float4* __restrict__ gsrc = EXPANDED ? p.geom_px : p.geom_pk;
    uint16_t* lcand = reinterpret_cast<uint16_t*>(lds_raw + p.lds_cand_off);
    unsigned char* lpath = lds_raw + p.lds_path_off;

    const int tid = threadIdx.x;
    const int lane = tid & 63;
    const int tid16 = (tid & ~63) | ((tid & 31) << 1) | ((tid >> 5) & 1);

    if (ISECT == 0) {
        for (uint32_t i = tid; i < p.n_sph_pad; i += BLOCK) lgeom[i] = gsrc[i];
        if (EXPANDED)
            for (uint32_t i = tid; i < p.n_sph_pad; i += BLOCK) lrr[i] = p.geom[i].w;
        __syncthreads();
    }

    if (LTREE) {
        float* ln = reinterpret_cast<float*>(lds_raw + p.lds_node_off);
        const uint32_t r0 = lt_r0(p.n_internal);
        for (uint32_t n = tid; n <= p.n_internal; n += BLOCK) {
            float* q = ln + LNODE_DW * n;
            if (n < p.n_internal) {
                const float4 a0 = p.trav[4u * n], a1 = p.trav[4u * n + 1], a2 = p.trav[4u * n + 2], a3 = p.trav[4u * n + 3];
                auto ref16 = [r0](uint32_t r) { return (r & LEAF_BIT) ? (0x8000u | (r & 0x7fffu)) : r0 + r * (uint32_t)LNODE_DW; };
                q[0] = a0.x; q[1] = a1.x; q[2] = a0.x;   q[3] = a2.x; q[4] = a3.x; q[5] = a2.x;
                q[6] = a0.y; q[7] = a1.y; q[8] = a0.y;   q[9] = a2.y; q[10] = a3.y; q[11] = a2.y;
                q[12] = a0.z; q[13] = a1.z; q[14] = a0.z; q[15] = a2.z; q[16] = a3.z; q[17] = a2.z;
                q[18] = __uint_as_float(ref16(__float_as_uint(a0.w)) | (ref16(__float_as_uint(a1.w)) << 16));
            } else {
                const float qn = __builtin_nanf(""), inf = __builtin_inff();
                for (int i = 0; i < 18; i++) q[i] = qn;
                for (int a = 0; a < 3; a++) { q[6 * a] = -inf; q[6 * a + 1] = inf; q[6 * a + 2] = -inf; }
                q[18] = __uint_as_float((r0 + p.n_internal * (uint32_t)LNODE_DW) * 0x10001u);
            }
        }
        float* nanf_ = ln + LNODE_DW * (p.n_internal + 1u);
        for (uint32_t i = tid; i < p.n_sph + p.n_tri + (uint32_t)LNODE_DW; i += BLOCK) nanf_[i] = __builtin_nanf("");
        __syncthreads();
    }
    const float* const lnodes = reinterpret_cast<const float*>(lds_raw + p.lds_node_off) - (LTREE ? (int)lt_r0(p.n_internal) : 0);
    const V3 corg = mk(p.org[0], p.org[1], p.org[2]);
    const V3 llc = mk(p.llc[0], p.llc[1], p.llc[2]);
    const V3 hor = mk(p.hor[0], p.hor[1], p.hor[2]);
    const V3 ver = mk(p.ver[0], p.ver[1], p.ver[2]);
    const bool exact_scan = (p.flags & 1u) != 0;
    const bool use_bvh = (p.flags & 2u) == 0;
    const float KMf = 1.0f - 0x1p-17f;
    const v2f NKM = {-KMf, -KMf};

    const uint32_t wave = (uint32_t)tid >> 6;
#define wq wave_q[wave]
#define wst wave_st[CAN_STAGE ? wave : 0u]
    float* const ring = p.ring + (size_t)(blockIdx.x * (uint32_t)(BLOCK / 64) + wave) * ((size_t)p.n_slots * p.slot_stride * 3u);
    const uint32_t all_free = p.n_slots >= 32u ? 0xffffffffu : (1u << p.n_slots) - 1u;
    uint32_t freem = all_free;
    uint32_t cur_slot = 0;
    uint32_t tile_u = 0, tile_units = 0;
    uint32_t tile_x0 = 0, tile_row = 0, tile_yg = 0;
    uint32_t tile_meta = STAGE_TILES << 16;
    uint64_t tile_seed = 0;
    bool q_drained = false;
    bool have_unit = false, need_ray = false;
    uint32_t useq = 0;
    Rng rng = {0, 0, 0, 0};
    uint32_t depth_left = 0, k = 0;
    V3 o = mk(0, 0, 0), d = mk(0, 0, 0);
    bool bounce = false;
    V3 bn = mk(0, 0, 0);
    float brough = 0.f;
    using Cnt = typename std::conditional<(ISECT >= 2), uint32_t, unsigned long long>::type;
    Cnt n_seg = 0, n_cand = 0, n_fall = 0;
    Cnt n_int = 0;
    Hit h;
    h.idx = -1;
    h.dist = 0.f;
    h.t = 0.f;
    RayAux aux = ray_aux(mk(1.f, 1.f, 1.f), false);
    auto AUX = [&]() -> RayAux { return QNODES ? ray_aux(d, (p.flags & 8u) != 0) : aux; };
    auto far_bound = [&](float best) -> float {
        float b = cull_bound(best, o, p.r_slack);
        if ((ISECT == 9 || ISECT == 6) && p.n_tri) b = __builtin_fmaxf(b, cull_bound_tri(best, o, p.tri_k, p.tri_diag, p.tri_es, p.tri_e));
        return b;
    };
    V3 td = mk(0, 0, 0);
    bool in_trav = false;
    uint32_t t_ref = 0, t_sp = 0, t_cnt = 0;
    uint32_t t_head = 0;
    V3 ig = mk(0, 0, 0), cq = mk(0, 0, 0);
    bool qfin = false;
    float t_far = __builtin_inff();
    uint32_t* lc32 = reinterpret_cast<uint32_t*>(lds_raw + p.lds_cand_off);
    uint32_t* lstack = reinterpret_cast<uint32_t*>(lds_raw + p.lds_stack_off);
    uint32_t sgx = 0, sgy = 0, sgz = 0;
    uint16_t* lc16 = reinterpret_cast<uint16_t*>(lds_raw + p.lds_cand_off);
    uint16_t* lstack16 = reinterpret_cast<uint16_t*>(lds_raw + p.lds_stack_off);

    if (BFSTEP) lstack16[tid16] = (uint16_t)(lt_r0(p.n_internal) + p.n_internal * (uint32_t)LNODE_DW);

    auto drain_counters = [&]() {
        const unsigned long long ws = wave_sum(n_seg), wc = wave_sum(n_cand), wf = wave_sum(n_fall);
        const unsigned long long wi = STATS ? wave_sum(n_int) : 0ull;
        if (lane == (int)__builtin_ctzll(__ballot(true))) {
            atomicAdd(&p.counters[0], ws);
            atomicAdd(&p.counters[1], wc);
            atomicAdd(&p.counters[2], wf);
            if (STATS) atomicAdd(&p.counters[3], wi);
        }
        n_seg = n_cand = n_fall = 0;
        n_int = 0;
    };
    const bool staging = CAN_STAGE && p.lds_stage_off != 0xffffffffu;
    unsigned char* const stage_base = lds_raw + (staging ? p.lds_stage_off + wave * (STAGE_TILES * STAGE_TILE_BYTES) : 0u);
    auto decode_tile = [&](uint32_t t, uint32_t& st, uint32_t& x0, uint32_t& row) {
        st = t / p.tiles_per_strip;
        const uint32_t rem = t - st * p.tiles_per_strip;
        row = rem / p.tiles_x;
        x0 = (rem - row * p.tiles_x) << 6;
    };
    auto div_spp = [&](uint32_t q) -> uint32_t { return p.spp_magic ? __umulhi(q, p.spp_magic) : q; };

    TDECL;
    for (;;) {
        WCOUNT(0);
        TSTAMP(5);
        TROUND;
        uint32_t px = 0, pyg = 0;
        if (freem != all_free) {
            __builtin_amdgcn_fence(__ATOMIC_ACQ_REL, "wavefront");
            const bool slot_done = (uint32_t)lane < SLOTS_MAX && (wq.cnt[cold<QNODES>(lane) & (int)(SLOTS_MAX - 1u)] & (SLOT_FREE | ((1u << SLOT_UNIT_BITS) - 1u))) == 0u;
            const uint32_t complete = (uint32_t)__ballot(slot_done);
            const uint32_t n_complete = (uint32_t)__builtin_popcount(complete);
            const bool issue_over = q_drained && tile_u == tile_units;
            if (n_complete >= p.commit_slots || (n_complete != 0u && ((uint32_t)__builtin_popcount(freem) < 2u || issue_over))) {
                WCOUNT(14);
                asm volatile("s_waitcnt vmcnt(0)" ::: "memory");
                const uint32_t n_lanes = p.n_slots * p.grp;
                for (uint32_t l0 = 0; l0 < n_lanes; l0 += 64u) {
                    const uint32_t L = l0 + (uint32_t)lane;
                    const uint32_t slot = p.grp == 1u ? L : __umulhi(L, p.grp_magic), g = L - slot * p.grp;
                    const bool mine = slot < p.n_slots && ((complete >> (slot & 31u)) & 1u) != 0u;
                    if (__ballot(mine) == 0ull) continue;
                    uint32_t stg = STAGE_TILES, cstrip = 0;
                    bool fin = false;
                    uint32_t pin = 0;
                    if (mine) {
                        const float* sb = ring + __umul24(slot, p.slot_stride) * 3u;
                        const uint32_t hx = ring_load(reinterpret_cast<const uint32_t*>(sb) + 0);
                        const uint32_t hrow = ring_load(reinterpret_cast<const uint32_t*>(sb) + 1);
                        const uint32_t hmeta = ring_load(reinterpret_cast<const uint32_t*>(sb) + 2);
                        const float* r = sb + 3u + g * p.upp * 3u;
                        float sum_r = 0.f, sum_g = 0.f, sum_b = 0.f;
                        cstrip = hmeta & 0xffu;
                        if (p.s_begin != 0u && g < ((hmeta >> 8) & 0xffu)) {
                            const float* a = p.strips[cstrip].acc + ((size_t)hrow * p.W + hx + g) * 3;
                            sum_r = a[0];
                            sum_g = a[1];
                            sum_b = a[2];
                        }
                        {
                            uint32_t i = 0;
                            auto batch = [&](auto cb_tag) {
                                constexpr int CB = decltype(cb_tag)::value;
#pragma clang loop unroll(disable)
                                for (; i + (uint32_t)CB <= p.upp; i += (uint32_t)CB) {
                                    LCOUNT(12);
                                    float c[3 * CB];
#pragma unroll
                                    for (int e = 0; e < 3 * CB; e++) c[e] = ring_load(r + e);
#pragma unroll
                                    for (int e = 0; e < CB; e++) {
                                        sum_r = sum_r + c[3 * e + 0];
                                        sum_g = sum_g + c[3 * e + 1];
                                        sum_b = sum_b + c[3 * e + 2];
                                    }
                                    r += 3 * CB;
                                }
                            };
                            if (RT_COMMIT_BATCH > 4 && !QNODES) batch(std::integral_constant<int, RT_COMMIT_BATCH>{});
                            batch(std::integral_constant<int, 4>{});
#pragma clang loop unroll(disable)
                            for (; i < p.upp; i++) {
                                LCOUNT(12);
                                const float cr = ring_load(r + 0);
                                const float cg = ring_load(r + 1);
                                const float cb = ring_load(r + 2);
                                sum_r = sum_r + cr;
                                sum_g = sum_g + cg;
                                sum_b = sum_b + cb;
                                r += 3;
                            }
                        }
                        if (g < ((hmeta >> 8) & 0xffu)) {
                            float cr_, cg_, cb_;
                            if (p.spp_rcp != 0.0f) {
                                cr_ = __builtin_sqrtf(sum_r * p.spp_rcp);
                                cg_ = __builtin_sqrtf(sum_g * p.spp_rcp);
                                cb_ = __builtin_sqrtf(sum_b * p.spp_rcp);
                            } else {
                                cr_ = __builtin_sqrtf(sum_r / p.spp_f);
                                cg_ = __builtin_sqrtf(sum_g / p.spp_f);
                                cb_ = __builtin_sqrtf(sum_b / p.spp_f);
                            }
                            const uint32_t sidx = hmeta & 0xffu;
                            stg = (hmeta >> 16) & 0xffu;
                            const size_t oidx = ((size_t)hrow * p.W + hx + g) * 3;
                            if (p.acc_out) {
                                float* a = p.strips[sidx].acc;
                                a[oidx + 0] = sum_r;
                                a[oidx + 1] = sum_g;
                                a[oidx + 2] = sum_b;
                            }
                            if (!CAN_STAGE || stg == STAGE_TILES) {
                                uint8_t* orgb = p.strips[sidx].rgb;
                                orgb[oidx + 0] = f32_as_u8(cr_ * 255.999f);
                                orgb[oidx + 1] = f32_as_u8(cg_ * 255.999f);
                                orgb[oidx + 2] = f32_as_u8(cb_ * 255.999f);
                            } else {
                                uint8_t* sd = stage_base + stg * STAGE_TILE_BYTES + ((hx + g) & 63u) * 3u;
                                sd[0] = f32_as_u8(cr_ * 255.999f);
                                sd[1] = f32_as_u8(cg_ * 255.999f);
                                sd[2] = f32_as_u8(cb_ * 255.999f);
                                fin = true;
                            }
                            float* of = p.strips[sidx].f32;
                            if (of) {
                                of[oidx + 0] = cr_;
                                of[oidx + 1] = cg_;
                                of[oidx + 2] = cb_;
                            }
                            (void)pin;
                        }
                    }
                    if (p.strip_cost && mine && g == 0u) {
                        const uint32_t sg = wq.cnt[slot & (SLOTS_MAX - 1u)] >> SLOT_UNIT_BITS;
                        if (cstrip == wq.cost_strip[0]) (void)__hip_atomic_fetch_add(&wq.cost_acc[0], sg, __ATOMIC_RELAXED, __HIP_MEMORY_SCOPE_WAVEFRONT);
                        else if (cstrip == wq.cost_strip[1]) (void)__hip_atomic_fetch_add(&wq.cost_acc[1], sg, __ATOMIC_RELAXED, __HIP_MEMORY_SCOPE_WAVEFRONT);
                        else if (sg) atomicAdd(&p.strip_cost[(blockIdx.x % COST_COPIES) * MAX_BATCH + cstrip], (unsigned long long)sg);
                    }
                    if (CAN_STAGE && __ballot(fin)) {
                        __builtin_amdgcn_fence(__ATOMIC_ACQ_REL, "wavefront");
#pragma unroll
                        for (uint32_t k = 0; k < STAGE_TILES; k++) {
                            const unsigned long long mk = __ballot(fin && stg == k);
                            if (mk == 0ull) continue;
                            const int left = (int)uni((uint32_t)wst.left[k]) - (int)__builtin_popcountll(mk);
                            if (left == 0) {
                                if (lane < (int)(STAGE_TILE_BYTES / 4)) {
                                    uint32_t* d32 = reinterpret_cast<uint32_t*>(((uintptr_t)uni(wst.dst_hi[k]) << 32) | uni(wst.dst_lo[k]));
                                    d32[lane] = reinterpret_cast<const uint32_t*>(stage_base + k * STAGE_TILE_BYTES)[lane];
                                }
                            }
                            if (lane == 0) wst.left[k] = left == 0 ? -1 : left;
                        }
                        __builtin_amdgcn_fence(__ATOMIC_ACQ_REL, "wavefront");
                    }
                }
                if (slot_done) wq.cnt[cold<QNODES>(lane)] = SLOT_FREE;
                freem = uni(freem | complete);
                __builtin_amdgcn_fence(__ATOMIC_ACQ_REL, "wavefront");
            }
        }
        TSTAMP(6);
        if (TRAVERSE && __ballot(((n_seg | n_cand | n_fall | n_int) & 0x80000000u) != 0)) drain_counters();
        {
            bool need = !have_unit;
            for (;;) {
                if (__ballot(need) == 0ull) break;
                if (tile_u == tile_units) {
                    if (q_drained) break;
                    uint32_t t = 0xffffffffu;
                    if (lane == 0) {
                        constexpr uint32_t WGC = (uint32_t)(BLOCK / 64) < (uint32_t)RT_QUEUE_TAKE_MIN ? (uint32_t)RT_QUEUE_TAKE_MIN : (uint32_t)(BLOCK / 64);
                        for (;;) {
                            const unsigned long long old = __hip_atomic_fetch_add(&wg_tiles, 1ull, __ATOMIC_RELAXED, __HIP_MEMORY_SCOPE_WORKGROUP);
                            if ((uint32_t)old < (uint32_t)(old >> 32)) {
                                t = (uint32_t)old;
                                break;
                            }
                            if (__hip_atomic_load(&wg_drained, __ATOMIC_RELAXED, __HIP_MEMORY_SCOPE_WORKGROUP)) break;
                            if (__hip_atomic_exchange(&wg_lock, 1u, __ATOMIC_ACQUIRE, __HIP_MEMORY_SCOPE_WORKGROUP) == 0u) {
                                const unsigned long long cur = __hip_atomic_load(&wg_tiles, __ATOMIC_RELAXED, __HIP_MEMORY_SCOPE_WORKGROUP);
                                bool done = false;
                                if ((uint32_t)cur >= (uint32_t)(cur >> 32)) {
                                    const uint32_t g = (uint32_t)atomicAdd(p.queue, (unsigned long long)WGC);
                                    if (g >= p.n_tiles) {
                                        __hip_atomic_store(&wg_drained, 1u, __ATOMIC_RELAXED, __HIP_MEMORY_SCOPE_WORKGROUP);
                                    } else {
                                        t = g;
                                        const uint32_t ge = min(g + WGC, p.n_tiles);
                                        __hip_atomic_store(&wg_tiles, (unsigned long long)(g + 1u) | ((unsigned long long)ge << 32),
                                                           __ATOMIC_RELAXED, __HIP_MEMORY_SCOPE_WORKGROUP);
                                    }
                                    done = true;
                                }
                                __hip_atomic_store(&wg_lock, 0u, __ATOMIC_RELEASE, __HIP_MEMORY_SCOPE_WORKGROUP);
                                if (done) break;
                            } else {
                                __builtin_amdgcn_s_sleep(2);
                            }
                        }
                    }
                    t = (uint32_t)__builtin_amdgcn_readfirstlane((int)t);
                    if (t == 0xffffffffu) {
                        q_drained = true;
                        TDRAINED;
                        break;
                    }
                    uint32_t sub = 0u, tw = 64u;
                    if (t >= p.tiles_big) {
                        const uint32_t e = t - p.tiles_big;
                        t = p.tiles_big + (e >> p.sub_shift);
                        tw = 64u >> p.sub_shift;
                        sub = (e & ((1u << p.sub_shift) - 1u)) * tw;
                    }
#ifndef RT_TILES_TOP_DOWN
                    t = p.tiles_total - 1u - t;
#endif
                    uint32_t tstrip;
                    decode_tile(t, tstrip, tile_x0, tile_row);
                    if (p.strip_cost && lane == 0 && (wq.cost_strip[0] != tstrip || wq.cost_acc[0] >= 0x80000000u)) {
                        if (wq.cost_acc[1]) atomicAdd(&p.strip_cost[(blockIdx.x % COST_COPIES) * MAX_BATCH + wq.cost_strip[1]], (unsigned long long)wq.cost_acc[1]);
                        wq.cost_acc[1] = wq.cost_acc[0];
                        wq.cost_strip[1] = wq.cost_strip[0];
                        wq.cost_acc[0] = 0u;
                        wq.cost_strip[0] = tstrip;
                    }
                    tile_x0 = uni(tile_x0 + sub);
                    tile_row = uni(tile_row);
                    if (tile_x0 >= p.W) continue;
                    tile_yg = uni(p.strips[tstrip].y0 + tile_row);
                    tile_seed = p.strips[tstrip].seed + (((uint64_t)tile_yg * p.W + tile_x0) * p.spp_all + p.s_begin) * (4ull * PHI);
                    tile_seed = (uint64_t)uni((uint32_t)tile_seed) | ((uint64_t)uni((uint32_t)(tile_seed >> 32)) << 32);
                    const uint32_t npix = min(tw, p.W - tile_x0);
                    tile_units = uni(npix * p.upp);
                    tile_u = 0u;
                    uint32_t tstage = STAGE_TILES;
                    if (staging && npix == 64u) {
                        uint8_t* dst = p.strips[tstrip].rgb + ((size_t)tile_row * p.W + tile_x0) * 3;
                        if ((reinterpret_cast<uintptr_t>(dst) & 3u) == 0) {
                            __builtin_amdgcn_fence(__ATOMIC_ACQ_REL, "wavefront");
                            for (uint32_t k = 0; k < STAGE_TILES; k++)
                                if ((int)uni((uint32_t)wst.left[k]) < 0) {
                                    tstage = k;
                                    break;
                                }
                            if (tstage < STAGE_TILES && lane == 0) {
                                wst.left[tstage] = 64;
                                wst.dst_lo[tstage] = (uint32_t)reinterpret_cast<uintptr_t>(dst);
                                wst.dst_hi[tstage] = (uint32_t)(reinterpret_cast<uintptr_t>(dst) >> 32);
                            }
                            __builtin_amdgcn_fence(__ATOMIC_ACQ_REL, "wavefront");
                        }
                    }
                    tile_meta = uni(tstrip | (tstage << 16));
                }
                bool got = false;
                uint32_t tv = 0;
                bool stall = false;
                {
                    const unsigned long long mask = __ballot(need);
                    const uint32_t want = (uint32_t)__builtin_popcountll(mask);
                    const uint32_t U = p.slot_stride - 1u;
                    const uint32_t k_open = __umulhi(tile_u + U - 1u, p.slotu_magic);
                    const uint32_t n_free = (uint32_t)__builtin_popcount(freem);
                    const uint32_t slot_room = (k_open + n_free) * U - tile_u;
                    const uint32_t take = min(want, min(tile_units - tile_u, slot_room));
                    stall = take < want && take == slot_room;
                    const uint32_t n_new = __umulhi(tile_u + take + U - 1u, p.slotu_magic) - k_open;
                    const uint32_t rank = __builtin_amdgcn_mbcnt_hi((uint32_t)(mask >> 32), __builtin_amdgcn_mbcnt_lo((uint32_t)mask, 0u));
                    got = need && rank < take;
                    tv = tile_u + rank;
                    const uint32_t k = __umulhi(tv, p.slotu_magic);
                    const uint32_t unit = tv - __umul24(k, U);
                    uint32_t m = freem;
                    for (uint32_t i = 0; i + 1u < n_new; i++) m = k > k_open + i ? (m & (m - 1u)) : m;
                    const uint32_t slot = k >= k_open ? (uint32_t)__builtin_ctz(m | 0x80000000u) : cur_slot;
                    if (got) {
                        useq = (slot << 24) | unit;
                        if (unit == 0u) {
                            const uint32_t un = min(U, tile_units - tv);
                            wq.cnt[slot] = un;
                            uint32_t* hdr = reinterpret_cast<uint32_t*>(ring + __umul24(slot, p.slot_stride) * 3u);
                            hdr[0] = tile_x0 + __umul24(k, p.grp);
                            hdr[1] = tile_row;
                            hdr[2] = (tile_meta & 0xffu) | (div_spp(un) << 8) | (tile_meta & 0xff0000u);
                        }
                    }
                    tile_u = uni(tile_u + take);
                    if (n_new) {
                        uint32_t fm = freem;
                        for (uint32_t i = 0; i + 1u < n_new; i++) fm &= fm - 1u;
                        cur_slot = uni((uint32_t)__builtin_ctz(fm));
                        freem = uni(fm & (fm - 1u));
                    }
                }
                TSTAMP(7);
                if (got) {
                    WCOUNT(1);
                    LCOUNT(0);
                    const uint32_t j = div_spp(tv);
                    px = tile_x0 + j;
                    pyg = tile_yg;
                    rng = seed_state(tile_seed + (uint64_t)(tv + __umul24(j, p.gap)) * (4ull * PHI));
                    have_unit = true;
                    need_ray = true;
                    bounce = false;
                    need = false;
                }
                if (stall) { LCOUNT(14); break; }
            }
        }
        const bool active = have_unit;
        if (!active) { LCOUNT(13); }
        TSTAMP(0);
        if (active && need_ray) {
            float x1, x2, sm;
            WCOUNT(2);
            for (;;) {
                WCOUNT(3);
                LCOUNT(1);
                x1 = uniform_m1_1(rng);
                x2 = uniform_m1_1(rng);
                sm = x1 * x1 + x2 * x2;
                if (bounce ? !(sm >= 1.0f) : (sm <= 1.0f)) break;
            }
            V3 xdir, pre, fallback;
            LCOUNT(2);
            if (bounce) {
                LCOUNT(3);
                const float factor = 2.0f * RT_SQRT(1.0f - sm);
                const V3 us = mk(x1 * factor, x2 * factor, 1.0f - 2.0f * sm);
                const V3 diffuse_dir = us + bn;
                const V3 glossy_dir = d - (2.0f * dot(d, bn)) * bn;
                pre = diffuse_dir + brough * (glossy_dir - diffuse_dir);
                fallback = bn;
            } else {
                LCOUNT(4);
                const V3 offset = lens_offset(p, x1, x2);
                const float u = ((float)px + gen_range_01(rng)) / p.u_den;
                const float v = ((float)(p.H - pyg - 1) + gen_range_01(rng)) / p.v_den;
                const V3 dir0 = normalize_or_zero(llc + u * hor + v * ver - corg);
                const V3 d1 = normalize(dir0);
                const V3 focal_point = corg + p.focus_distance * d1;
                o = corg + offset;
                pre = focal_point - o;
                fallback = mk(0.f, 0.f, 0.f);
                depth_left = p.depth;
                k = 0;
            }
            if (!try_normalize(pre, xdir)) xdir = fallback;
            d = normalize(xdir);
            need_ray = false;
            bounce = false;
        }
        TSTAMP(1);
        const bool wave_busy = __ballot(active) != 0ull || freem != all_free || !q_drained || tile_u != tile_units;
        if (STREAMED) {
            if (!__syncthreads_or(wave_busy ? 1 : 0)) break;
        } else {
            if (!wave_busy) break;
        }

        if (active && !in_trav) {
            h.idx = -1;
            aux = ray_aux(d, (p.flags & 8u) != 0);
            if (!TRAVERSE) td = 2.0f * d;
            n_seg++;
            if (QNODES) {
                const V3 og = mk((o.x - p.q_base[0]) * p.q_rstep[0], (o.y - p.q_base[1]) * p.q_rstep[1], (o.z - p.q_base[2]) * p.q_rstep[2]);
                ig = mk(p.q_step[0] * aux.inv.x, p.q_step[1] * aux.inv.y, p.q_step[2] * aux.inv.z);
                cq = mk(-(og.x * ig.x), -(og.y * ig.y), -(og.z * ig.z));
                const float big = 0x1p100f, tiny = 0x1p-60f;
                const float ax = __builtin_fabsf(ig.x), ay = __builtin_fabsf(ig.y), az = __builtin_fabsf(ig.z);
                qfin = aux.finite && ax < big && ay < big && az < big && ax > tiny && ay > tiny && az > tiny &&
                       __builtin_fabsf(og.x) < 0x1p18f && __builtin_fabsf(og.y) < 0x1p18f && __builtin_fabsf(og.z) < 0x1p18f;
            }
            if (LTREE) {
                aux.finite = aux.finite && __builtin_fabsf(o.x) < __builtin_inff() && __builtin_fabsf(o.y) < __builtin_inff() &&
                             __builtin_fabsf(o.z) < __builtin_inff();
                sgx = aux.sx ? 1u : 0u;
                sgy = aux.sy ? 1u : 0u;
                sgz = aux.sz ? 1u : 0u;
            }
            if (CULL) {
                t_far = __builtin_inff();
                for (uint32_t j = 0; j < p.n_big; j++) {
                    const uint32_t prim = p.big[j];
                    float t;
                    bool hit;
                    if (prim < p.n_sph) {
                        const float4 g = RT_SPHERE_REC(p, prim);
                        hit = exact_sphere(o, 2.0f * d, mk(g.x, g.y, g.z), g.w, p.t_min, p.t_max, t);
                    } else {
                        hit = exact_triangle(o, d, p.tri + 9 * (size_t)(prim - p.n_sph), p.t_min, p.t_max, t);
                    }
                    if (hit)
                        consider_if<true>(h, (int)prim, o, d, t, [&]() { return bvh_reaches(p.bvh_nodes, p.leaf_of[prim], o, AUX()); }, p.leaf_of);
                }
                if (h.idx >= 0) t_far = far_bound(h.dist);
            }
            if (TRAVERSE) {
                t_ref = p.root_ref;
                t_sp = BFSTEP ? 1u : 0u;
                t_cnt = 0;
                in_trav = (p.n_sph + p.n_tri) > 0;
            }
        }
        if constexpr (TRAVERSE) {
            auto root_test = [&](uint32_t i) {
                    LCOUNT(6);
                    const uint32_t prim = LTREE ? (uint32_t)lc16[i * BLOCK + tid16] & 0x7fffu
                                          : p.list16 ? (uint32_t)lc16[i * BLOCK + tid16] : lc32[i * BLOCK + tid];
                    float t;
                    if (prim < p.n_sph) {
                        const float4 g = RT_SPHERE_REC(p, prim);
                        if (exact_sphere(o, 2.0f * d, mk(g.x, g.y, g.z), g.w, p.t_min, p.t_max, t)) {
                            if (QNODES)
                                consider_if<CULL>(h, (int)prim, o, d, t, [&]() {
                                    if (!qfin || (p.n_sph + p.n_tri) == 1) return true;
                                    const float4 s = at32(p.geom_r, prim);
                                    return intersects_aabb_finite(o, AUX(), make_float4(s.x - s.w, s.y - s.w, s.z - s.w, 0.f),
                                                                  make_float4(s.x + s.w, s.y + s.w, s.z + s.w, 0.f));
                                }, p.leaf_of);
                            else if (CULL)
                                consider<1>(h, (int)prim, o, d, t, aux, p.bvh_nodes, p.leaf_of);
                            else
                                consider<0>(h, (int)prim, o, d, t, aux, p.bvh_nodes, p.leaf_of);
                        }
                    } else {
                        if (exact_triangle(o, d, p.tri + 9 * (size_t)(prim - p.n_sph), p.t_min, p.t_max, t)) {
                            if (QNODES)
                                consider_if(h, (int)prim, o, d, t,
                                            [&]() { return !qfin || bvh_reaches(p.bvh_nodes, p.leaf_of[prim], o, AUX()); });
                            else if (CULL)
                                consider<1>(h, (int)prim, o, d, t, aux, p.bvh_nodes, p.leaf_of);
                            else
                                consider<0>(h, (int)prim, o, d, t, aux, p.bvh_nodes, p.leaf_of);
                        }
                    }
            };
            auto flush = [&]() {
                if (BFSTEP) n_cand += t_cnt - t_head;
#pragma clang loop unroll(disable)
                for (uint32_t i = BFSTEP ? t_head : 0u; i < t_cnt; i++) root_test(i);
                t_cnt = 0;
                if (BFSTEP) t_head = 0;
                if (CULL && h.idx >= 0) t_far = far_bound(h.dist);
            };
            auto flush_one = [&]() {
                n_cand++;
                root_test(t_head);
                t_head++;
                if (t_head == t_cnt) t_head = t_cnt = 0;
                if (CULL && h.idx >= 0) t_far = far_bound(h.dist);
            };

            constexpr bool COMPACT = XNODES;
            auto flush_c = [&](bool want) {
                const uint32_t cnt = want ? t_cnt : 0u;
                uint32_t excl = 0, total = 0;
#pragma unroll
                for (int b = 0; b < 4; b++) {
                    const unsigned long long m = __ballot(((cnt >> b) & 1u) != 0);
                    excl += (uint32_t)__builtin_amdgcn_mbcnt_hi((uint32_t)(m >> 32), __builtin_amdgcn_mbcnt_lo((uint32_t)m, 0u)) << b;
                    total += (uint32_t)__builtin_popcountll(m) << b;
                }
                const unsigned long long act = __ballot(true);
                const uint32_t n_act = (uint32_t)__builtin_popcountll(act);
                const uint32_t rank = (uint32_t)__builtin_amdgcn_mbcnt_hi((uint32_t)(act >> 32), __builtin_amdgcn_mbcnt_lo((uint32_t)act, 0u));
                uint32_t* const w_pref = reinterpret_cast<uint32_t*>(lds_raw + p.lds_cmp_off) + (tid >> 6) * 256;
                float* const w_dist = reinterpret_cast<float*>(w_pref + 64);
                float* const w_root = reinterpret_cast<float*>(w_pref + 128);
                uint32_t* const w_hit = w_pref + 192;
                w_pref[rank] = excl | ((uint32_t)lane << 16);
                __builtin_amdgcn_fence(__ATOMIC_ACQ_REL, "wavefront");
                int best_k = -1;
                float best_t = 0.f;
                auto own_prim = [&](uint32_t k) -> uint32_t {
                    return p.list16 ? (uint32_t)lc16[k * BLOCK + tid16] : lc32[k * BLOCK + tid];
                };
                for (uint32_t base = 0; base < total; base += n_act) {
                    const uint32_t j = base + rank;
                    const bool valid = j < total;
                    uint32_t R = 0, ent = w_pref[0];
                    if (valid) {
#pragma unroll
                        for (uint32_t stp = 32; stp > 0; stp >>= 1) {
                            const uint32_t c = R + stp;
                            if (c < n_act) {
                                const uint32_t e = w_pref[c];
                                if ((e & 0xffffu) <= j) { R = c; ent = e; }
                            }
                        }
                    }
                    const uint32_t L = ent >> 16, slot = j - (ent & 0xffffu);
                    const V3 ro = mk(__shfl(o.x, (int)L, 64), __shfl(o.y, (int)L, 64), __shfl(o.z, (int)L, 64));
                    const V3 rd = mk(__shfl(d.x, (int)L, 64), __shfl(d.y, (int)L, 64), __shfl(d.z, (int)L, 64));
                    bool hit = false;
                    float t = 0.f, dist = 0.f;
                    if (valid) {
                        LCOUNT(6);
                        const uint32_t ot = ((uint32_t)tid & ~63u) | L;
                        const uint32_t ot16 = (ot & ~63u) | ((ot & 31u) << 1) | ((ot >> 5) & 1u);
                        const uint32_t prim = p.list16 ? (uint32_t)lc16[slot * BLOCK + ot16] : lc32[slot * BLOCK + ot];
                        if (prim < p.n_sph) {
                            const float4 g = RT_SPHERE_REC(p, prim);
                            hit = exact_sphere(ro, 2.0f * rd, mk(g.x, g.y, g.z), g.w, p.t_min, p.t_max, t);
                        } else {
                            hit = exact_triangle(ro, rd, p.tri + 9 * (size_t)(prim - p.n_sph), p.t_min, p.t_max, t);
                        }
                        if (hit) {
                            const V3 pp = ro + t * rd;
                            dist = vlength(pp - ro);
                        }
                    }
                    w_dist[rank] = dist;
                    w_root[rank] = t;
                    w_hit[rank] = hit ? 1u : 0u;
                    __builtin_amdgcn_fence(__ATOMIC_ACQ_REL, "wavefront");
                    if (cnt) {
                        const uint32_t k0 = excl > base ? excl : base, k1 = min(excl + cnt, base + n_act);
#pragma clang loop unroll(disable)
                        for (uint32_t k = k0; k < k1; k++) {
                            if (!w_hit[k - base]) continue;
                            const float dk = w_dist[k - base];
                            bool take = best_k < 0 ? (h.idx < 0 || h.dist > dk) : (h.dist > dk);
                            if (CULL && !take && h.dist == dk && (best_k >= 0 || h.idx >= 0)) {
                                const uint32_t cur = best_k >= 0 ? own_prim((uint32_t)best_k) : (uint32_t)h.idx;
                                take = p.leaf_of[own_prim(k - excl)] < p.leaf_of[cur];
                            }
                            if (take) {
                                h.dist = dk;
                                best_k = (int)(k - excl);
                                best_t = w_root[k - base];
                            }
                        }
                    }
                    __builtin_amdgcn_fence(__ATOMIC_ACQ_REL, "wavefront");
                }
                if (best_k >= 0) {
                    h.idx = (int)own_prim((uint32_t)best_k);
                    h.t = best_t;
                }
                if (want) t_cnt = 0;
                if (CULL && want && h.idx >= 0) t_far = far_bound(h.dist);
            };
            auto push = [&](uint32_t v) {
                if (LTREE) lstack16[t_sp * BLOCK + tid16] = (uint16_t)v;
                else if (!CAPPED || t_sp < p.stack_lds) lstack[t_sp * BLOCK + tid] = v;
                else p.stack_ovf[(size_t)(t_sp - p.stack_lds) * p.ovf_stride + (blockIdx.x * BLOCK + tid)] = v;
                t_sp++;
            };
            auto pop = [&]() -> uint32_t {
                --t_sp;
                if (LTREE) return (uint32_t)lstack16[t_sp * BLOCK + tid16];
                if (!CAPPED || t_sp < p.stack_lds) return lstack[t_sp * BLOCK + tid];
                return p.stack_ovf[(size_t)(t_sp - p.stack_lds) * p.ovf_stride + (blockIdx.x * BLOCK + tid)];
            };
            if constexpr (BFSTEP) {
            const uint32_t DONE = lt_r0(p.n_internal) + p.n_internal * (uint32_t)LNODE_DW;
            constexpr int STEPS = RT_STEPS_PER_CHECK_LTREE;
            static_assert(MAXL_LTREE > STEPS, "the leaf list must take a block of appends");
            constexpr uint32_t SLOT = (uint32_t)BLOCK * 2u;
            typedef __attribute__((address_space(3))) unsigned char lds_byte;
            typedef __attribute__((address_space(3))) uint16_t lds_u16;
            const uint32_t lds0 = (uint32_t)(uintptr_t)(lds_byte*)lds_raw;
            const uint32_t stack0_a = lds0 + p.lds_stack_off + (uint32_t)tid16 * 2u;
// ... 262 lines not shown
            for (;;) {
                if (seg_active) h.idx = -1;
                for (uint32_t ch = 0; ch < p.n_chunks; ch++) {
                    const uint32_t base = ch * p.chunk;
                    const uint32_t cn = min(p.chunk, p.n_sph_pad - base);
                    if (STREAMED) {
                        __syncthreads();
                        for (uint32_t i = tid; i < cn; i += BLOCK) lgeom[i] = gsrc[base + i];
                        if (EXPANDED)
                            for (uint32_t i = tid; i < cn; i += BLOCK) lrr[i] = p.geom[base + i].w;
                        __syncthreads();
                    }
                    if (seg_active) {
                        uint32_t cnt = 0;
                        if (!exact_scan) {
                            uint32_t ncand_it = 0;
                            v2f k0x, k0y, k0z, k1x, k1y, k1z, kA, kB;
                            if (EXPANDED) {
                                const float A = __builtin_fmaf(d.z, o.z, __builtin_fmaf(d.y, o.y, d.x * o.x));
                                const float oo =
                                    __builtin_fmaf(o.z, o.z, __builtin_fmaf(o.y, o.y, o.x * o.x)) * (1.0f - 0x1p-16f);
                                k0x = v2f{-d.x, -d.x}; k0y = v2f{-d.y, -d.y}; k0z = v2f{-d.z, -d.z};
                                k1x = v2f{-2.0f * o.x, -2.0f * o.x}; k1y = v2f{-2.0f * o.y, -2.0f * o.y};
                                k1z = v2f{-2.0f * o.z, -2.0f * o.z};
                                kA = v2f{A, A};
                                kB = v2f{oo, oo};
                            } else {
                                k0x = v2f{o.x, o.x}; k0y = v2f{o.y, o.y}; k0z = v2f{o.z, o.z};
                                k1x = v2f{d.x, d.x}; k1y = v2f{d.y, d.y}; k1z = v2f{d.z, d.z};
                                kA = NKM;
                                kB = NKM;
                            }
                            for (uint32_t j = 0; j < cn; j += UNROLL) {
                                float t[UNROLL];
    #pragma unroll
                                for (int q = 0; q < UNROLL / 2; q++) {
                                    const float4 A4 = lgeom[j + 2 * q];
                                    const float4 B4 = lgeom[j + 2 * q + 1];
                                    const v2f cx = {A4.x, A4.y}, cy = {A4.z, A4.w}, cz = {B4.x, B4.y}, cw = {B4.z, B4.w};
                                    v2f tt;
                                    if (EXPANDED) {
                                        const v2f bb = pk_fma(k0x, cx, pk_fma(k0y, cy, pk_fma(k0z, cz, kA)));
                                        const v2f qq = pk_fma(k1x, cx, pk_fma(k1y, cy, pk_fma(k1z, cz, cw + kB)));
                                        tt = pk_fma(bb, bb, -qq);
                                    } else {
                                        const v2f ocx = k0x - cx, ocy = k0y - cy, ocz = k0z - cz;
                                        const v2f bb = pk_fma(k1z, ocz, pk_fma(k1y, ocy, k1x * ocx));
                                        const v2f l2 = pk_fma(ocz, ocz, pk_fma(ocy, ocy, ocx * ocx));
                                        tt = pk_fma(l2, kA, pk_fma(bb, bb, cw));
                                    }
                                    t[2 * q] = tt.x;
                                    t[2 * q + 1] = tt.y;
                                }
                                const float m = __builtin_fmaxf(
                                    __builtin_fmaxf(__builtin_fmaxf(t[0], t[1]), __builtin_fmaxf(t[2], t[3])),
                                    __builtin_fmaxf(__builtin_fmaxf(t[4], t[5]), __builtin_fmaxf(t[6], t[7])));
                                if (!(m < 0.0f)) {
                                    WCOUNT(4);
                                    uint32_t neg = 0;
    #pragma unroll
                                    for (int q = 0; q < UNROLL; q++) neg |= (__float_as_uint(t[q]) >> 31) << q;
                                    const uint32_t pass8 = ~neg & 0xffu;
                                    if (cnt < (uint32_t)MAXC) lcand[cnt * BLOCK + tid] = (uint16_t)(((j >> 3) << 8) | pass8);
                                    cnt++;
                                    ncand_it += (uint32_t)__builtin_popcount(pass8);
                                }
                            }
                            if (!inline_chain) n_cand += ncand_it;
                        }
                        const bool direct = exact_scan || cnt > (uint32_t)MAXC;
                        if (!exact_scan && direct && !inline_chain) n_fall++;
                        const uint32_t n_ent = direct ? (cn >> 3) : cnt;
                        uint32_t ei = 0, grp = 0, bits = 0;
                        for (;;) {
                            if (bits == 0) {
                                if (ei == n_ent) break;
                                if (direct) {
                                    grp = ei;
                                    bits = 0xffu;
                                } else {
                                    const uint32_t e = lcand[ei * BLOCK + tid];
                                    grp = e >> 8;
                                    bits = e & 0xffu;
                                }
                                ei++;
                                if (bits == 0) continue;
                            }
                            WCOUNT(5);
                            const uint32_t j = grp * 8 + (uint32_t)__builtin_ctz(bits);
                            bits &= bits - 1;
                            const uint32_t fo = (j >> 1) * 8 + (j & 1);
                            const V3 cen = mk(lgeomf[fo], lgeomf[fo + 2], lgeomf[fo + 4]);
                            const float rr = EXPANDED ? lrr[j] : lgeomf[fo + 6];
                            float t;
                            if (exact_sphere(o, td, cen, rr, p.t_min, p.t_max, t)) {
                                WCOUNT(6);
                                if (!use_bvh) {
                                    if (p.world_rank) consider<1>(h, (int)(base + j), o, d, t, aux, p.bvh_nodes, p.world_rank);
                                    else consider<0>(h, (int)(base + j), o, d, t, aux, p.bvh_nodes, p.leaf_of);
                                } else if (inline_chain)
                                    consider<2>(h, (int)(base + j), o, d, t, aux, p.bvh_nodes, p.leaf_of);
                                else
                                    consider<1>(h, (int)(base + j), o, d, t, aux, p.bvh_nodes, p.leaf_of);
                            }
                        }
                    }
                }
                if (seg_active) {
                    for (uint32_t j = 0; j < p.n_tri; j++) {
                        if (use_bvh && p.n_sph + p.n_tri > 1 &&
                            !intersects_aabb(o, aux, p.tri_box[2 * (size_t)j], p.tri_box[2 * (size_t)j + 1]))
                            continue;
                        float t;
                        if (exact_triangle(o, d, p.tri + 9 * (size_t)j, p.t_min, p.t_max, t)) {
                            if (!use_bvh) {
                                if (p.world_rank) consider<1>(h, (int)(p.n_sph + j), o, d, t, aux, p.bvh_nodes, p.world_rank);
                                else consider<0>(h, (int)(p.n_sph + j), o, d, t, aux, p.bvh_nodes, p.leaf_of);
                            } else if (inline_chain)
                                consider<2>(h, (int)(p.n_sph + j), o, d, t, aux, p.bvh_nodes, p.leaf_of);
                            else
                                consider<1>(h, (int)(p.n_sph + j), o, d, t, aux, p.bvh_nodes, p.leaf_of);
                        }
                    }
                }
                bool redo = false;
                if (seg_active && use_bvh && !inline_chain && h.idx >= 0) {
                    WCOUNT(7);
                    redo = !bvh_reaches(p.bvh_nodes, p.leaf_of[h.idx], o, aux);
                }
                if (STREAMED) {
                    if (!__syncthreads_or(redo ? 1 : 0)) break;
                } else {
                    if (!redo) break;
                }
                seg_active = redo;
                inline_chain = true;
            }
        }
        if (active && !in_trav) {
            float term_r, term_g, term_b;
            bool finished;
            LCOUNT(7);
            const bool hit = h.idx >= 0;
            float em = 0.f;
            float4 m = make_float4(0.f, 0.f, 0.f, 0.f);
            V3 hp = o, nv = d;
            if (hit) {
                WCOUNT(8);
                LCOUNT(8);
                em = at32(p.emis, (uint32_t)h.idx);
                m = at32(p.mat, (uint32_t)h.idx);
                if (!(em > 0.0f)) {
                    hp = o + h.t * d;
                    if ((uint32_t)h.idx < p.n_sph) {
                        float4 g = TRAVERSE ? RT_SPHERE_REC(p, (uint32_t)h.idx) : at32(p.geom, (uint32_t)h.idx);
                        nv = hp - mk(g.x, g.y, g.z);
                    } else {
                        const float* tv = p.tri + 9 * (size_t)(h.idx - p.n_sph);
                        V3 A = mk(tv[0], tv[1], tv[2]), B = mk(tv[3], tv[4], tv[5]), C = mk(tv[6], tv[7], tv[8]);
                        nv = cross(A - B, A - C);
                    }
                }
            }
            const V3 nn = normalize_or_zero(nv);
            if (hit) {
                if (em > 0.0f) {
                    term_r = m.x * em;
                    term_g = m.y * em;
                    term_b = m.z * em;
                    finished = true;
                } else {
                    const V3 n = nn;
                    if (p.path32)
                        reinterpret_cast<uint32_t*>(lpath)[k * BLOCK + cold<QNODES>(tid)] = (uint32_t)h.idx;
                    else
                        reinterpret_cast<uint16_t*>(lpath)[k * BLOCK + cold<QNODES>(tid16)] = (uint16_t)h.idx;
                    k++;
                    depth_left--;
                    if (depth_left == 0) {
                        WCOUNT(9);
                        for (;;) {
                            WCOUNT(10);
                            const float y1 = uniform_m1_1(rng);
                            const float y2 = uniform_m1_1(rng);
                            if (!(y1 * y1 + y2 * y2 >= 1.0f)) break;
                        }
                    } else {
                        o = hp;
                        bn = n;
                        brough = m.w;
                        bounce = true;
                        need_ray = true;
                    }
                    finished = (depth_left == 0);
                    term_r = term_g = term_b = 0.0f;
                }
            } else {
                WCOUNT(11);
                LCOUNT(9);
                float t = nn.y * 0.5f + 1.0f;
                float omt = 1.0f - t;
                term_r = 1.0f * t + 0.3f * omt;
                term_g = 1.0f * t + 0.3f * omt;
                term_b = 1.0f * t + 0.8f * omt;
                finished = true;
            }
            if (finished) {
                WCOUNT(12);
                LCOUNT(10);
                {
                    auto path_idx = [&](uint32_t i) -> uint32_t {
                        return p.path32 ? reinterpret_cast<uint32_t*>(lpath)[i * BLOCK + cold<QNODES>(tid)]
                                        : (uint32_t) reinterpret_cast<uint16_t*>(lpath)[i * BLOCK + cold<QNODES>(tid16)];
                    };
                    uint32_t i = k;
#pragma clang loop unroll(disable)
                    while (i >= 2) {
                        WCOUNT(13);
                        LCOUNT(11);
                        const float4 ma = at32(p.mat, path_idx(i - 1)), mb = at32(p.mat, path_idx(i - 2));
                        term_r = mb.x * (ma.x * term_r);
                        term_g = mb.y * (ma.y * term_g);
                        term_b = mb.z * (ma.z * term_b);
                        i -= 2;
                    }
                    if (i) {
                        WCOUNT(13);
                        LCOUNT(11);
                        const float4 ma = at32(p.mat, path_idx(0));
                        term_r = ma.x * term_r;
                        term_g = ma.y * term_g;
                        term_b = ma.z * term_b;
                    }
                }
                {
                    const uint32_t slot = useq >> 24;
                    float* r = ring + (__umul24(slot, p.slot_stride) + 1u + (useq & 0xffffffu)) * 3u;
                    r[0] = term_r;
                    r[1] = term_g;
                    r[2] = term_b;
                    const uint32_t usegs = k + ((hit && !(em > 0.0f)) ? 0u : 1u);
                    (void)__hip_atomic_fetch_add(&wq.cnt[slot], (usegs << SLOT_UNIT_BITS) - 1u, __ATOMIC_RELAXED, __HIP_MEMORY_SCOPE_WAVEFRONT);
                    have_unit = false;
                }
            }
        }
        TSTAMP(4);
    }

    if (p.strip_cost && lane < 2 && wq.cost_acc[lane])
        atomicAdd(&p.strip_cost[(blockIdx.x % COST_COPIES) * MAX_BATCH + wq.cost_strip[lane]], (unsigned long long)wq.cost_acc[lane]);
    drain_counters();
    TFLUSH;
#undef wq
#undef wst
}

using KernelFn = void (*)(const KParams);
KernelFn kernel_linear(int isect, bool expanded);
KernelFn kernel_traverse(int isect, bool stats);
void sqrt_selftest_launch(uint32_t from, unsigned long long n, unsigned long long* d_bad, hipStream_t st);

}
```

### ray_tracer_s8_amd/csrc/rt_kernels_trav.hip

```cpp
#include "rt_kernel.hip.h"

namespace rtk {
template <bool STATS>
KernelFn traverse_kernel(int isect) {
    switch (isect) {
        case 5: return rt_tile_kernel<5, false, LTREE_BLOCK, STATS>;
        case 6: return rt_tile_kernel<6, false, LTREE_BLOCK, STATS>;
        case 7: return rt_tile_kernel<7, false, BLOCK, STATS>;
        case 8: return rt_tile_kernel<8, false, BLOCK, STATS>;
        case 9: return rt_tile_kernel<9, false, BLOCK, STATS>;
        case 3: return rt_tile_kernel<3, false, BLOCK, STATS>;
        case 2: return rt_tile_kernel<2, false, BLOCK, STATS>;
        case 4: return rt_tile_kernel<4, false, BLOCK, STATS>;
        default: return nullptr;
    }
}
KernelFn kernel_traverse(int isect, bool stats) { return stats ? traverse_kernel<true>(isect) : traverse_kernel<false>(isect); }

__global__ void sqrt_selftest_kernel(uint32_t from, unsigned long long n, unsigned long long* bad) {
    unsigned long long mine = 0;
    for (unsigned long long i = blockIdx.x * (unsigned long long)blockDim.x + threadIdx.x; i < n; i += (unsigned long long)gridDim.x * blockDim.x) {
        float x = __uint_as_float(from + (uint32_t)i);
        asm volatile("" : "+v"(x));
        const float ref = __builtin_sqrtf(x);
        const float a = sqrt_rn(x), b = sqrt_rn<true>(x);
        const bool both_nan_a = (a != a) && (ref != ref), both_nan_b = (b != b) && (ref != ref);
        if (__float_as_uint(a) != __float_as_uint(ref) && !both_nan_a) mine++;
        if (__float_as_uint(b) != __float_as_uint(ref) && !both_nan_b) mine++;
    }
    if (mine) atomicAdd(bad, mine);
}
void sqrt_selftest_launch(uint32_t from, unsigned long long n, unsigned long long* d_bad, hipStream_t st) {
    hipLaunchKernelGGL(sqrt_selftest_kernel, dim3(4096), dim3(256), 0, st, from, n, d_bad);
}
}

#ifdef RT_DEBUG_HOOKS
#define RT_UNIT_ID 1
#include "rt_unit.hip.h"
#endif
```

### ray_tracer_s8_amd/csrc/rt_plan.h

```cpp
#pragma once
#include <algorithm>
#include <cmath>
#include <cstddef>
#include <cstdint>
#include <vector>

#include "rt_consts.h"
#include "rt_tile.h"

namespace rtplan {

constexpr size_t LDS_LIMIT = 160 * 1024 - 3072;
constexpr uint32_t RESIDENT_MAX = rtk::CHUNK;
constexpr uint32_t STREAM_CHUNK = 2048;
constexpr uint32_t STACK_LDS_MAX = 12;
constexpr uint32_t RT_QNODES_MIN_PRIMS = 4096;
constexpr uint32_t DENSE_SCAN_MAX_PRIMS = 192;
constexpr float DENSE_SCAN_MIN_DENSITY = 3.0f;
constexpr float DENSE_MID_MIN_DENSITY = 2.5f;
constexpr uint32_t DENSE_MID_MIN_PRIMS = 512;
constexpr float FIELD_MID_MIN_DENSITY = 0.15f;
constexpr float LT_CULL_MIN_DENSITY = 2.2f;
constexpr uint32_t TRAVERSE_MIN_PRIMS = 2;

struct SceneShape {
    uint32_t n_sph = 0, n_sph_pad = 0, n_tri = 0;
    uint32_t bvh_depth = 0, n_internal = 0;
    uint32_t root_ref = 0;
    float cull_density = 0.f;
    bool cull_pays = false;
    bool xcull_pays = false;
    bool quant_ok = false;
    bool tri_ok = false;
    float r_slack = 0.f;
    bool inverted_boxes = false;
    bool expanded = false;
    float leaf_density = 0.f;
};

struct Knobs {
    int lds_tree = 1;
    int cull_walk = -1;
    int no_stage = 0;
    int slots = 0;
    int commit_slots = 0;
    int force_capped = 0;
    int stack_lds = 0;
    int compact = 1;
    int refill_eighths = 0;
    int tail_tiles = -1;
};

struct Engine {
    int isect, isect_capped, block;
};
constexpr Engine ENGINES[8] = {
    {0, -1, rtk::BLOCK},
    {1, -1, rtk::BLOCK},
    {2, -1, rtk::BLOCK},
    {3, 4, rtk::BLOCK},
    {5, -1, rtk::LTREE_BLOCK},
    {7, 8, rtk::BLOCK},
    {9, -1, rtk::BLOCK},
    {6, -1, rtk::LTREE_BLOCK},
};
constexpr int N_ISECT = 10;

struct SampleRange {
    uint32_t begin, end;
    bool pass;
};

struct Plan {
    int status = RT_OK;
    const char* error = nullptr;
    int engine = 0;
    bool capped = false;
    int isect = 0;
    int block = rtk::BLOCK;
    bool expanded = false;
    bool count_steps = false;
    size_t lds = 0;
    uint32_t maxl_l2 = 0;
    uint32_t ovf_entries = 0;
    uint32_t blocks = 0;
    size_t ring_bytes = 0;
    size_t ovf_words = 0;
};

inline bool cull_wanted(uint32_t flags, int knob, bool rule) {
    return (flags & RT_FLAG_NO_CULL_WALK) ? false : (flags & RT_FLAG_CULL_WALK) ? true : knob >= 0 ? knob != 0 : rule;
}

struct Pose {
    float origin[3];
    float u[3], v[3], w[3];
};

inline float length3(const float a[3]) { return std::sqrt((a[0] * a[0] + a[1] * a[1]) + a[2] * a[2]); }
inline void cross3(const float a[3], const float b[3], float out[3]) {
    out[0] = a[1] * b[2] - a[2] * b[1];
    out[1] = a[2] * b[0] - a[0] * b[2];
    out[2] = a[0] * b[1] - a[1] * b[0];
}

inline bool make_pose(const rt_camera& c, Pose& ps) {
    if (c.flags != 0 || c.reserved != 0) return false;
    for (int i = 0; i < 3; i++)
        if (!std::isfinite(c.origin[i]) || !std::isfinite(c.target[i]) || !std::isfinite(c.up[i])) return false;
    Pose r;
    float d[3], x[3];
    for (int i = 0; i < 3; i++) d[i] = c.origin[i] - c.target[i];
    const float ld = length3(d);
    if (!(ld > 0.0f) || !std::isfinite(ld)) return false;
    for (int i = 0; i < 3; i++) r.w[i] = d[i] / ld;
    cross3(c.up, r.w, x);
    const float lx = length3(x);
    if (!(lx > 0.0f) || !std::isfinite(lx)) return false;
    for (int i = 0; i < 3; i++) r.u[i] = x[i] / lx;
    cross3(r.w, r.u, r.v);
    for (int i = 0; i < 3; i++) r.origin[i] = c.origin[i];
    ps = r;
    return true;
}

template <class KP>
auto set_lens(KP& p, const float lu[3], const float lv[3], int) -> decltype((void)p.lens_u[0]) {
    for (int i = 0; i < 3; i++) {
        p.lens_u[i] = lu[i];
        p.lens_v[i] = lv[i];
    }
}
template <class KP>
void set_lens(KP&, const float*, const float*, long) {}

template <class KP>
void fill_camera(const rt_tile_request& rq, KP& p) {
    const float origin[3] = {0.f, 0.f, 0.f};
    const float aspect_ratio = (float)rq.width / (float)rq.height;
    const float image_height = (float)rq.height;
    const float vh = 2.0f * std::tan(rq.fov / 2.0f);
    const float vw = aspect_ratio * vh;
    const float hor[3] = {vw, 0.f, 0.f}, ver[3] = {0.f, vh, 0.f};
    const float foc[3] = {0.f, 0.f, rq.focal_length};
    for (int i = 0; i < 3; i++) {
        p.org[i] = origin[i];
        p.hor[i] = hor[i];
        p.ver[i] = ver[i];
        float v = origin[i] - hor[i] / 2.0f;
        v = v - ver[i] / 2.0f;
        v = v - foc[i];
        p.llc[i] = v;
    }
    p.lens_radius = rq.aperture / 2.0f;
    const float lens_u[3] = {p.lens_radius, 0.f, 0.f}, lens_v[3] = {0.f, p.lens_radius, 0.f};
    set_lens(p, lens_u, lens_v, 0);
    p.focus_distance = rq.focus_distance;
    p.u_den = aspect_ratio * image_height - 1.0f;
    p.v_den = image_height - 1.0f;
}

template <class KP>
void fill_camera(const rt_tile_request& rq, const Pose& ps, KP& p) {
    const float aspect_ratio = (float)rq.width / (float)rq.height;
    const float image_height = (float)rq.height;
    const float vh = 2.0f * std::tan(rq.fov / 2.0f);
    const float vw = aspect_ratio * vh;
    p.lens_radius = rq.aperture / 2.0f;
    float lens_u[3], lens_v[3];
    for (int i = 0; i < 3; i++) {
        const float hor = vw * ps.u[i], ver = vh * ps.v[i], foc = rq.focal_length * ps.w[i];
        p.org[i] = ps.origin[i];
        p.hor[i] = hor;
        p.ver[i] = ver;
        float v = ps.origin[i] - hor / 2.0f;
        v = v - ver / 2.0f;
        v = v - foc;
        p.llc[i] = v;
        lens_u[i] = p.lens_radius * ps.u[i];
        lens_v[i] = p.lens_radius * ps.v[i];
    }
    set_lens(p, lens_u, lens_v, 0);
    p.focus_distance = rq.focus_distance;
    p.u_den = aspect_ratio * image_height - 1.0f;
    p.v_den = image_height - 1.0f;
}

template <class KP>
void fill_camera(const rt_tile_request& rq, const Pose* pose, KP& p) {
    if (pose) fill_camera(rq, *pose, p);
    else fill_camera(rq, p);
}

template <class KP>
Plan plan_launch(const SceneShape& sh, const rt_tile_request& rq, uint32_t n_strips, const SampleRange& smp, const Knobs& kn, KP& p,
                 const Pose* pose = nullptr) {
    using namespace rtk;
    Plan pl;
    p.W = rq.width;
    p.H = rq.height;
    p.Hs = rq.height / rq.divisions;
    const uint32_t s_begin = smp.begin, s_end = smp.end;
    p.upp = s_end - s_begin;
    p.spp_all = rq.spp;
    p.s_begin = s_begin;
    p.gap = rq.spp - p.upp;
    p.acc_out = smp.pass ? 1u : 0u;
    p.depth = rq.max_bounces + 1;
    p.n_sph = sh.n_sph;
    p.n_sph_pad = sh.n_sph_pad;
    p.n_tri = sh.n_tri;
    p.flags = rq.flags;
    if (sh.inverted_boxes) p.flags |= RT_FLAG_FULL_CHAIN;
    const uint32_t fl = rq.flags;
    const uint32_t n_prims = sh.n_sph + sh.n_tri;
    const bool trav_ok = !(fl & (RT_FLAG_EXACT_SCAN | RT_FLAG_NO_BVH_CULL | RT_FLAG_LINEAR_SCAN)) &&
                         sh.bvh_depth < (uint32_t)TRAV_STACK && n_prims > 0;
    const bool dense_pile = sh.n_tri == 0 && n_prims <= DENSE_SCAN_MAX_PRIMS && sh.cull_density >= DENSE_SCAN_MIN_DENSITY;
    const bool traverse = trav_ok && ((fl & RT_FLAG_BVH_TRAVERSE) || (n_prims >= TRAVERSE_MIN_PRIMS && !dense_pile));
    bool ltree_fits = false;
    const size_t lt_lane = ((size_t)MAXL_LTREE + (size_t)(rq.max_bounces + 1) + (size_t)(sh.bvh_depth + 2)) * sizeof(uint16_t);
    if (traverse && kn.lds_tree != 0 && !(fl & RT_FLAG_NO_LDS_TREE) && sh.n_internal > 0 && n_prims <= 0x7fffu &&
        ((size_t)sh.n_internal + 2) * LNODE_DW < 0x8000u) {
        const size_t fixed = (((size_t)sh.n_internal + 2) * LNODE_DW + n_prims) * 4 + 16 + lt_lane * LTREE_BLOCK;
        ltree_fits = fixed <= LDS_LIMIT;
    }
    const bool dense_mid = sh.cull_pays && !(fl & RT_FLAG_NO_CULL_WALK) && !ltree_fits && sh.cull_density >= DENSE_MID_MIN_DENSITY &&
                           n_prims >= DENSE_MID_MIN_PRIMS;
    const bool field_mid = !ltree_fits && sh.n_tri == 0 && n_prims < RT_QNODES_MIN_PRIMS && sh.cull_density >= FIELD_MID_MIN_DENSITY;
    const bool qnodes = traverse && sh.quant_ok && !(fl & RT_FLAG_EXACT_NODES) &&
                        ((fl & RT_FLAG_QUANT_NODES) || (n_prims >= RT_QNODES_MIN_PRIMS && sh.n_tri <= sh.n_sph) || dense_mid ||
                         field_mid);
    const bool ltree = ltree_fits && !qnodes;
    const bool cull = qnodes && cull_wanted(fl, kn.cull_walk, sh.cull_pays) && sh.n_tri == 0 && std::isfinite(sh.r_slack);
    const bool xcull = traverse && !qnodes && !ltree && cull_wanted(fl, kn.cull_walk, sh.xcull_pays) && sh.n_tri > 0 && sh.tri_ok &&
                       std::isfinite(sh.r_slack) && !sh.inverted_boxes;
    const bool lt_cull_ok = ltree && !sh.inverted_boxes && std::isfinite(sh.r_slack) && (sh.n_tri == 0 || sh.tri_ok);
    const bool ltcull = lt_cull_ok && cull_wanted(fl, kn.cull_walk, sh.cull_density >= LT_CULL_MIN_DENSITY);
    const bool streamed = !traverse && sh.n_sph_pad > RESIDENT_MAX;
    pl.engine = traverse ? (ltree ? (ltcull ? 7 : 4) : qnodes ? (cull ? 5 : 3) : xcull ? 6 : 2) : (streamed ? 1 : 0);
    const int bs = ENGINES[pl.engine].block;
    p.chunk = traverse ? 0 : (streamed ? STREAM_CHUNK : sh.n_sph_pad);
    p.n_chunks = p.chunk ? (sh.n_sph_pad + p.chunk - 1) / p.chunk : 0;
    p.path32 = (sh.n_sph + sh.n_tri) > 65536u ? 1u : 0u;
    size_t geom_bytes = traverse ? 0 : (size_t)(p.chunk ? p.chunk : 1) * 4 * sizeof(float);
    p.lds_cand_off = (uint32_t)geom_bytes;
    size_t path_bytes = (size_t)p.depth * BLOCK * (p.path32 ? 4 : 2);
    const bool want_stage = kn.no_stage == 0 && ((traverse && !ltree) || streamed);
    const bool list16 = traverse && !ltree && n_prims <= 65536u;
    const size_t stage_bytes_wg = (size_t)STAGE_TILES * STAGE_TILE_BYTES * (bs / 64);
    const uint32_t stack_capped = sh.bvh_depth + 1;
    const uint32_t stack_need = sh.bvh_depth + (ltree ? 2u : 1u);
    uint32_t maxl = qnodes ? (uint32_t)MAXL : (uint32_t)MAXL_EXACT, stack_lds = stack_need;
    if (traverse && qnodes) {
        const size_t per_wg = (160u * 1024u - 4096u) / 5u - 512u;
        const size_t slot = (size_t)BLOCK * (list16 ? sizeof(uint16_t) : sizeof(uint32_t));
        const size_t fixed = path_bytes + (size_t)stack_need * BLOCK * sizeof(uint32_t) + (want_stage ? stage_bytes_wg : 0);
        if (kn.force_capped == 0 && fixed + (size_t)MINL * slot <= per_wg) {
            maxl = (uint32_t)std::min<size_t>((size_t)MAXL, (per_wg - fixed) / slot);
        } else {
            const uint32_t cap = kn.stack_lds > 0 ? (uint32_t)kn.stack_lds : STACK_LDS_MAX;
            pl.capped = stack_capped > cap;
            stack_lds = pl.capped ? cap : stack_need;
        }
    }
    p.maxl = maxl;
    p.stack_lds = stack_lds;
    p.list16 = list16 ? 1u : 0u;
    size_t cand_bytes = traverse ? (size_t)maxl * BLOCK * (list16 ? sizeof(uint16_t) : sizeof(uint32_t))
                                 : (size_t)MAXC * BLOCK * sizeof(uint16_t);
    p.lds_path_off = (uint32_t)(geom_bytes + cand_bytes);
    const bool expanded = !traverse && sh.expanded && !(fl & RT_FLAG_OC_BROAD_PHASE);
    p.lds_rr_off = (uint32_t)(geom_bytes + cand_bytes + path_bytes);
    size_t rr_bytes = expanded ? (size_t)(p.chunk ? p.chunk : 1) * sizeof(float) : 0;
    p.lds_stack_off = (uint32_t)(geom_bytes + cand_bytes + path_bytes + rr_bytes);
    size_t stack_bytes = traverse ? (size_t)stack_lds * BLOCK * sizeof(uint32_t) : 0;
    size_t lds = geom_bytes + cand_bytes + path_bytes + rr_bytes + stack_bytes;
    p.n_internal = sh.n_internal;
    p.lds_node_off = 0;
    if (ltree) {
        size_t off = ((((size_t)sh.n_internal + 2) * LNODE_DW + n_prims) * 4 + 15) & ~(size_t)15;
        p.lds_cand_off = (uint32_t)off;
        uint32_t lt_maxl = MAXL_LTREE;
        while (lt_maxl < (uint32_t)MAXL_LTREE_MAX &&
               off + ((size_t)(lt_maxl + 1) + p.depth + stack_need) * bs * sizeof(uint16_t) <= LDS_LIMIT) lt_maxl++;
        p.maxl = lt_maxl;
        off += (size_t)lt_maxl * bs * sizeof(uint16_t);
        p.lds_path_off = (uint32_t)off;
        off += (size_t)p.depth * bs * sizeof(uint16_t);
        p.lds_stack_off = (uint32_t)off;
        off += (size_t)stack_need * bs * sizeof(uint16_t);
        lds = off;
    }
    p.lds_cmp_off = 0xffffffffu;
    if (traverse && !qnodes && !ltree && kn.compact != 0 && lds + 1024u * (BLOCK / 64) + 16 <= LDS_LIMIT) {
        lds = (lds + 15) & ~(size_t)15;
        p.lds_cmp_off = (uint32_t)lds;
        lds += 1024u * (BLOCK / 64);
    }
    p.lds_stage_off = 0xffffffffu;
    if (want_stage && lds + stage_bytes_wg <= LDS_LIMIT) {
        lds = (lds + 15) & ~(size_t)15;
        p.lds_stage_off = (uint32_t)lds;
        lds += stage_bytes_wg;
    }
    pl.lds = lds;
    if (lds > LDS_LIMIT) {
        pl.status = RT_ERR_LIMIT;
        pl.error = "LDS budget exceeded (scene chunk + path stack)";
        return pl;
    }
    pl.isect = pl.capped ? ENGINES[pl.engine].isect_capped : ENGINES[pl.engine].isect;
    pl.block = bs;
    pl.expanded = expanded;
    pl.count_steps = traverse && (fl & RT_FLAG_COUNT_STEPS);
    pl.maxl_l2 = maxl;
    pl.ovf_entries = pl.capped ? stack_capped - stack_lds : 0u;
    fill_camera(rq, pose, p);
    p.t_min = rq.t_min;
    p.t_max = rq.t_max;
    p.spp_f = (float)s_end;
    p.spp_rcp = (s_end & (s_end - 1u)) == 0u ? 1.0f / (float)s_end : 0.0f;
    p.root_ref = sh.root_ref;
    if (ltree) p.root_ref = (p.root_ref & LEAF_BIT) ? (0x8000u | (p.root_ref & 0x7fffu)) : lt_r0(sh.n_internal) + p.root_ref * (uint32_t)LNODE_DW;
    p.refill_eighths = kn.refill_eighths > 0 ? (uint32_t)kn.refill_eighths : (n_prims >= RT_QNODES_MIN_PRIMS ? 4u : 2u);
    p.n_strips = n_strips;
    p.tiles_x = (p.W + 63u) / 64u;
    p.tiles_per_strip = p.tiles_x * p.Hs;
    {
        p.grp = p.upp >= 8u ? 1u : (8u + p.upp - 1u) / p.upp;
        const uint64_t slot_units = (uint64_t)p.grp * p.upp;
        p.grp_magic = p.grp > 1u ? (uint32_t)((1ull << 32) / p.grp) + 1u : 0u;
        p.slot_stride = 1u + (uint32_t)slot_units;
        const uint64_t fewest = slot_units <= 256u ? 16u : slot_units <= 1024u ? 8u : 4u;
        p.n_slots = kn.slots > 0 ? std::min<uint32_t>((uint32_t)kn.slots, SLOTS_MAX)
                                 : (uint32_t)std::min<uint64_t>(SLOTS_MAX, std::max<uint64_t>(fewest, 384u / slot_units));
        const uint32_t cs = kn.commit_slots > 0 ? (uint32_t)kn.commit_slots : std::max<uint32_t>(1u, p.n_slots / 4u);
        p.commit_slots = std::min<uint32_t>(cs, p.n_slots);
        p.spp_magic = p.upp > 1u ? (uint32_t)((1ull << 32) / p.upp) + 1u : 0u;
        p.slotu_magic = (uint32_t)((1ull << 32) / slot_units) + 1u;
    }
    const uint64_t n_tiles = (uint64_t)p.tiles_per_strip * n_strips;
    if (n_tiles > 0x1fffffffull) {
        pl.status = RT_ERR_LIMIT;
        pl.error = "too many tiles in one launch";
        return pl;
    }
    p.tiles_total = (uint32_t)n_tiles;
    p.n_tiles = (uint32_t)n_tiles;
    p.tiles_big = (uint32_t)n_tiles;
    return pl;
}

template <class KP>
void plan_queue(Plan& pl, uint32_t blocks, const Knobs& kn, KP& p) {
    const uint32_t waves_per_wg = (uint32_t)pl.block / 64u;
    const uint32_t useful = (p.n_tiles + waves_per_wg - 1) / waves_per_wg;
    if (blocks > useful) blocks = useful ? useful : 1;
    pl.blocks = blocks;
    const uint64_t waves = (uint64_t)blocks * waves_per_wg;
    const bool all_parts = p.tiles_total < 16ull * waves || p.upp > 16u;
    const uint64_t conv = std::min<uint64_t>(p.tiles_total, kn.tail_tiles >= 0 ? (uint64_t)kn.tail_tiles : all_parts ? (uint64_t)p.tiles_total : 2ull * waves);
    p.sub_shift = p.upp > 32u ? 4u : 2u;
    if ((((uint64_t)p.tiles_total - conv) + (conv << p.sub_shift)) > 0x7fffffffull) p.sub_shift = 2u;
    p.tiles_big = p.tiles_total - (uint32_t)conv;
    p.n_tiles = p.tiles_big + ((uint32_t)conv << p.sub_shift);
    p.ovf_stride = blocks * (uint32_t)pl.block;
    pl.ovf_words = (size_t)pl.ovf_entries * p.ovf_stride;
    pl.ring_bytes = (size_t)blocks * waves_per_wg * p.n_slots * p.slot_stride * 12u;
}

constexpr int QUERY_BLOCK = 256;

struct QueryPlan {
    int engine = 2;
    int scan_mode = 2;
    bool full_chain = false;
    size_t lds = 0;
};

inline QueryPlan plan_query(const SceneShape& sh, uint32_t flags) {
    QueryPlan q;
    const uint32_t n_prims = sh.n_sph + sh.n_tri;
    const bool no_cull = (flags & RT_FLAG_NO_BVH_CULL) != 0;
    const bool walk = !no_cull && !(flags & (RT_FLAG_EXACT_SCAN | RT_FLAG_LINEAR_SCAN)) && n_prims > 0 &&
                      sh.bvh_depth < (uint32_t)rtk::TRAV_STACK;
    q.engine = walk ? 2 : 1;
    q.scan_mode = no_cull ? 0 : 2;
    q.full_chain = (flags & RT_FLAG_FULL_CHAIN) != 0 || sh.inverted_boxes;
    q.lds = walk ? ((size_t)sh.bvh_depth + 1) * QUERY_BLOCK * sizeof(uint32_t) : 0;
    return q;
}

constexpr uint32_t DIRECT_MAX_LIGHTS = 1u << 23;

struct DirectPlan {
    QueryPlan query;
    bool too_many = false;
};

inline DirectPlan plan_direct(const SceneShape& sh, uint32_t n_lights, uint32_t flags) {
    DirectPlan d;
    d.query = plan_query(sh, flags);
    d.too_many = n_lights > DIRECT_MAX_LIGHTS;
    return d;
}

using NeePlan = DirectPlan;

inline NeePlan plan_nee(const SceneShape& sh, uint32_t n_lights, uint32_t flags) { return plan_direct(sh, n_lights, flags); }

constexpr uint32_t TRACE_LDS_CU = 160 * 1024;
constexpr uint32_t TRACE_BLOCKS[] = {256, 128, 64};

struct TracePlan {
    int engine = 2;
    int scan_mode = 2;
    bool full_chain = false;
    uint32_t block = 256;
    bool path32 = false;
    size_t lds_path_off = 0;
    size_t lds = 0;
};

inline TracePlan plan_trace(const SceneShape& sh, uint32_t flags, uint32_t max_bounces) {
    const QueryPlan q = plan_query(sh, flags);
    TracePlan t;
    t.engine = q.engine;
    t.scan_mode = q.scan_mode;
    t.full_chain = q.full_chain;
    t.path32 = (sh.n_sph + sh.n_tri) > 65536u;
    const size_t stack_lane = q.engine == 2 ? ((size_t)sh.bvh_depth + 1) * sizeof(uint32_t) : 0;
    const size_t path_lane = ((size_t)max_bounces + 1) * (t.path32 ? 4 : 2);
    for (uint32_t b : TRACE_BLOCKS) {
        t.block = b;
        if (2 * (stack_lane + path_lane) * b <= TRACE_LDS_CU) break;
    }
    t.lds_path_off = stack_lane * t.block;
    t.lds = (stack_lane + path_lane) * t.block;
    return t;
}

constexpr uint32_t DN_TILE_X = 64, DN_TILE_Y = 4, DN_BLOCK = DN_TILE_X * DN_TILE_Y;
constexpr uint32_t DN_MAX_ITER = 8;
constexpr uint32_t DN_LDS_MAX_STEP = 2;
constexpr size_t DN_LDS_CU = 160 * 1024;
constexpr uint32_t DN_WG_PER_CU_MAX = 8;
constexpr size_t DN_REC = 16;
constexpr size_t DN_ALIGN = 256;

struct DenoisePlan {
    uint64_t npix = 0;
    uint32_t tiles_x = 0;
    size_t off_guide = 0;
    size_t off_color[2] = {0, 0};
    size_t scratch_bytes = 0;
    uint32_t step[DN_MAX_ITER] = {};
    size_t lds[DN_MAX_ITER] = {};
    uint32_t wg_per_cu[DN_MAX_ITER] = {};
};

inline size_t dn_align(size_t b) { return (b + DN_ALIGN - 1) / DN_ALIGN * DN_ALIGN; }

inline size_t dn_window_bytes(uint32_t s, bool guided) {
    return (size_t)(DN_TILE_X + 4 * s) * (DN_TILE_Y + 4 * s) * DN_REC * (guided ? 2 : 1);
}

inline DenoisePlan plan_denoise(uint32_t W, uint32_t R, uint32_t iterations, bool guided, uint32_t lds_max_step = DN_LDS_MAX_STEP) {
    DenoisePlan p;
    p.npix = (uint64_t)W * R;
    p.tiles_x = (W + DN_TILE_X - 1) / DN_TILE_X;
    const size_t buf = dn_align((size_t)p.npix * DN_REC);
    p.off_guide = 0;
    p.off_color[0] = buf;
    p.off_color[1] = 2 * buf;
    p.scratch_bytes = 3 * buf;
    for (uint32_t i = 0; i < iterations && i < DN_MAX_ITER; i++) {
        const uint32_t s = 1u << i;
        p.step[i] = s;
        const size_t b = dn_window_bytes(s, guided);
        if (s <= lds_max_step && b <= DN_LDS_CU) {
            p.lds[i] = b;
            p.wg_per_cu[i] = (uint32_t)std::min<size_t>(DN_WG_PER_CU_MAX, DN_LDS_CU / b);
        } else {
            p.wg_per_cu[i] = DN_WG_PER_CU_MAX;
        }
    }
    return p;
}

enum : unsigned { STAGE_UP = 1, STAGE_DOWN = 2, STAGE_DEVICE = 4 };
struct StageEntry {
    const void* host;
    size_t bytes;
    unsigned copy;
    size_t off;
    bool present() const { return host || (copy & STAGE_DEVICE); }
};
inline size_t stage_layout(StageEntry* e, size_t n) {
    size_t top = 0;
    for (size_t k = 0; k < n; k++) {
        e[k].off = top;
        if (e[k].present()) top += dn_align(e[k].bytes);
// ... 27 lines not shown
```

Measured before the change: 15820.

## Add sphere-only and plain-frame specializations of the LDS-tree traversal kernels

Adds a TRIS template parameter so LDS-tree kernels can be instantiated without triangle handling, selected when the scene has no triangles. This removes triangle branches, the triangle cull bound and the 32-bit path entries from the hot path. It also adds a 'plain' commit path for the common case of no accumulation, no f32 output, power-of-two spp and one pixel per lane, which drops the accumulator reads and per-lane grouping math. The cost is more kernel instantiations and a larger binary. The host must pick the right variant, and a wrong pick would give incorrect results.

```diff
diff --git a/ray_tracer_s8_amd/csrc/rt_api.hip b/ray_tracer_s8_amd/csrc/rt_api.hip
--- a/ray_tracer_s8_amd/csrc/rt_api.hip
+++ b/ray_tracer_s8_amd/csrc/rt_api.hip
@@ -114,13 +114,18 @@
     DBG_TAIL_TILES,
     DBG_STRIP_COST,
     DBG_DENOISE_LDS_STEP,
+    DBG_LTREE_GENERAL,
+    DBG_PLAIN_FRAME,
     DBG_N
 };
 std::atomic<int> g_dbg[DBG_N];
 const struct { const char* env; int def; } g_dbg_spec[DBG_N] = {
     {"RT_LDS_TREE", 1}, {"RT_CULL_WALK", -1}, {"RT_NO_STAGE", 0}, {"RT_SLOTS", 0}, {"RT_FORCE_CAPPED", 0},
     {"RT_STACK_LDS", 0}, {"RT_COMPACT", 1}, {"RT_REFILL_EIGHTHS", 0}, {"RT_COMMIT_SLOTS", 0}, {"RT_VERBOSE", 0}, {"RT_REORDER", 1}, {"RT_TAIL_TILES", -1}, {"RT_STRIP_COST", 1},
-    {"RT_DENOISE_LDS_STEP", -1}};
+    {"RT_DENOISE_LDS_STEP", -1}, {"RT_LTREE_GENERAL", 0}, {"RT_PLAIN_FRAME", 1}};
+#ifdef RT_DEBUG_HOOKS
+std::atomic<int> g_last_variant{0};
+#endif
 std::once_flag g_dbg_once;
 void dbg_load_env() {
     std::call_once(g_dbg_once, [] {
@@ -151,6 +156,8 @@
     k.compact = dbg(DBG_COMPACT);
     k.refill_eighths = dbg(DBG_REFILL_EIGHTHS);
     k.tail_tiles = dbg(DBG_TAIL_TILES);
+    k.ltree_general = dbg(DBG_LTREE_GENERAL);
+    k.plain_frame = dbg(DBG_PLAIN_FRAME);
     return k;
 }
 
@@ -349,8 +356,11 @@
     p.counters = sc->d_counters.get();
     p.queue = sc->d_counters.get() + 4 + sc->events.pending().size();
     p.strip_cost = dbg(DBG_STRIP_COST) ? d_strip_cost : nullptr;
-
-    const rtk::KernelFn kern = pl.isect < 2 ? rtk::kernel_linear(pl.isect, pl.expanded) : rtk::kernel_traverse(pl.isect, pl.count_steps);
+    bool any_f32 = false;
+    for (uint32_t i = 0; i < n; i++) any_f32 = any_f32 || p.strips[i].f32 != nullptr;
+    p.plain = rtplan::plain_frame(pl, any_f32, p.strip_cost != nullptr) ? 1u : 0u;
+
+    const rtk::KernelFn kern = pl.isect < 2 ? rtk::kernel_linear(pl.isect, pl.expanded) : rtk::kernel_traverse(pl.isect, pl.count_steps, pl.tris);
     int per_cu = 0;
     HIPCHK(hipOccupancyMaxActiveBlocksPerMultiprocessor(&per_cu, kern, pl.block, pl.lds));
     if (per_cu < 1) per_cu = 1;
@@ -376,6 +386,9 @@
     HIPCHK(hipMemsetAsync(p.queue, 0, sizeof(unsigned long long), stream));
     sc->last_engine = (uint32_t)pl.engine;
     sc->last_form = pl.expanded ? 1u : 0u;
+#ifdef RT_DEBUG_HOOKS
+    g_last_variant.store((pl.tris ? 0 : 1) | (p.plain ? 2 : 0), std::memory_order_relaxed);
+#endif
     if ((rc = enqueue(sc, stream, kern, pl.blocks, pl.block, pl.lds, p))) return rc;
     HIPCHK(hipEventRecord(rg->buf.done.get(), stream));
     if (p.stack_ovf) HIPCHK(hipEventRecord(sc->stack_ovf.done.get(), stream));
@@ -652,6 +665,10 @@
         for (int alt = 0; alt < 2; alt++)
             HIPCHK(hipFuncSetAttribute((const void*)(isect < 2 ? rtk::kernel_linear(isect, alt != 0) : rtk::kernel_traverse(isect, alt != 0)),
                                        hipFuncAttributeMaxDynamicSharedMemorySize, (int)rtplan::LDS_LIMIT));
+    for (int isect : {5, 6})
+        for (int alt = 0; alt < 2; alt++)
+            HIPCHK(hipFuncSetAttribute((const void*)rtk::kernel_traverse(isect, alt != 0, false), hipFuncAttributeMaxDynamicSharedMemorySize,
+                                       (int)rtplan::LDS_LIMIT));
     Stream st, cs;
     HIPCHK(st.create(hipStreamNonBlocking));
     HIPCHK(cs.create(hipStreamNonBlocking));
@@ -1714,6 +1731,7 @@
 extern "C" __attribute__((visibility("default"))) int rt_debug_set(const char* name, int value) {
     dbg_load_env();
     if (!name) return INT32_MIN;
+    if (!strcmp(name, "RT_LAST_VARIANT")) return g_last_variant.exchange(value);
     for (int k = 0; k < DBG_N; k++)
         if (!strcmp(name, g_dbg_spec[k].env)) return g_dbg[k].exchange(value);
     return INT32_MIN;
diff --git a/ray_tracer_s8_amd/csrc/rt_kernel.hip.h b/ray_tracer_s8_amd/csrc/rt_kernel.hip.h
--- a/ray_tracer_s8_amd/csrc/rt_kernel.hip.h
+++ b/ray_tracer_s8_amd/csrc/rt_kernel.hip.h
@@ -142,6 +142,7 @@
     unsigned long long* counters;
     unsigned long long* queue;
     StripDesc strips[MAX_BATCH];
+    uint32_t plain;
 };
 
 struct V3 {
@@ -496,7 +497,7 @@
     return cull_bound_tri(best, o.x, o.y, o.z, k, diag, es, e);
 }
 
-template <int ISECT, bool EXPANDED, int BS = BLOCK, bool STATS = false>
+template <int ISECT, bool EXPANDED, int BS = BLOCK, bool STATS = false, bool TRIS = true>
 __global__ __launch_bounds__(BS, (ISECT == 5 || ISECT == 6) ? RT_MINWAVES_LTREE : ISECT == 9 ? RT_MINWAVES_TRAV : ISECT >= 7 ? RT_MINWAVES_CULL : ISECT >= 3 ? RT_MINWAVES_QTRAV : ISECT == 2 ? RT_MINWAVES_TRAV : RT_MINWAVES) void rt_tile_kernel(const KParams p) {
     constexpr int BLOCK = BS;
     constexpr bool STREAMED = (ISECT == 1);
@@ -508,6 +509,9 @@
     constexpr bool LTREE = (ISECT == 5 || ISECT == 6);
     constexpr uint32_t LB = LTREE ? 0x8000u : LEAF_BIT;
     constexpr bool BFSTEP = LTREE;
+    static_assert(TRIS || LTREE, "the sphere-only instantiation exists for the LDS-tree kernels");
+    constexpr bool PLAIN_OK = LTREE;
+    auto path32 = [&]() -> bool { return !LTREE && p.path32 != 0u; };
     const uint32_t ML = QNODES ? p.maxl : (uint32_t)MAXL_EXACT;
     extern __shared__ __attribute__((aligned(16))) unsigned char lds_raw[];
     __shared__ unsigned long long wg_tiles;
@@ -613,7 +617,7 @@
     auto AUX = [&]() -> RayAux { return QNODES ? ray_aux(d, (p.flags & 8u) != 0) : aux; };
     auto far_bound = [&](float best) -> float {
         float b = cull_bound(best, o, p.r_slack);
-        if ((ISECT == 9 || ISECT == 6) && p.n_tri) b = __builtin_fmaxf(b, cull_bound_tri(best, o, p.tri_k, p.tri_diag, p.tri_es, p.tri_e));
+        if (TRIS && (ISECT == 9 || ISECT == 6) && p.n_tri) b = __builtin_fmaxf(b, cull_bound_tri(best, o, p.tri_k, p.tri_diag, p.tri_es, p.tri_e));
         return b;
     };
     V3 td = mk(0, 0, 0);
@@ -668,127 +672,132 @@
             if (n_complete >= p.commit_slots || (n_complete != 0u && ((uint32_t)__builtin_popcount(freem) < 2u || issue_over))) {
                 WCOUNT(14);
                 asm volatile("s_waitcnt vmcnt(0)" ::: "memory");
-                const uint32_t n_lanes = p.n_slots * p.grp;
-                for (uint32_t l0 = 0; l0 < n_lanes; l0 += 64u) {
-                    const uint32_t L = l0 + (uint32_t)lane;
-                    const uint32_t slot = p.grp == 1u ? L : __umulhi(L, p.grp_magic), g = L - slot * p.grp;
-                    const bool mine = slot < p.n_slots && ((complete >> (slot & 31u)) & 1u) != 0u;
-                    if (__ballot(mine) == 0ull) continue;
-                    uint32_t stg = STAGE_TILES, cstrip = 0;
-                    bool fin = false;
-                    uint32_t pin = 0;
-                    if (mine) {
-                        const float* sb = ring + __umul24(slot, p.slot_stride) * 3u;
-                        const uint32_t hx = ring_load(reinterpret_cast<const uint32_t*>(sb) + 0);
-                        const uint32_t hrow = ring_load(reinterpret_cast<const uint32_t*>(sb) + 1);
-                        const uint32_t hmeta = ring_load(reinterpret_cast<const uint32_t*>(sb) + 2);
-                        const float* r = sb + 3u + g * p.upp * 3u;
-                        float sum_r = 0.f, sum_g = 0.f, sum_b = 0.f;
-                        cstrip = hmeta & 0xffu;
-                        if (p.s_begin != 0u && g < ((hmeta >> 8) & 0xffu)) {
-                            const float* a = p.strips[cstrip].acc + ((size_t)hrow * p.W + hx + g) * 3;
-                            sum_r = a[0];
-                            sum_g = a[1];
-                            sum_b = a[2];
-                        }
-                        {
-                            uint32_t i = 0;
-                            auto batch = [&](auto cb_tag) {
-                                constexpr int CB = decltype(cb_tag)::value;
+                auto commit_complete = [&](auto plain_tag) {
+                    constexpr bool PLAIN = decltype(plain_tag)::value;
+                    const uint32_t n_lanes = PLAIN ? p.n_slots : p.n_slots * p.grp;
+                    for (uint32_t l0 = 0; l0 < n_lanes; l0 += 64u) {
+                        const uint32_t L = l0 + (uint32_t)lane;
+                        const uint32_t slot = (PLAIN || p.grp == 1u) ? L : __umulhi(L, p.grp_magic), g = PLAIN ? 0u : L - slot * p.grp;
+                        const bool mine = slot < p.n_slots && ((complete >> (slot & 31u)) & 1u) != 0u;
+                        if (__ballot(mine) == 0ull) continue;
+                        uint32_t stg = STAGE_TILES, cstrip = 0;
+                        bool fin = false;
+                        uint32_t pin = 0;
+                        if (mine) {
+                            const float* sb = ring + __umul24(slot, p.slot_stride) * 3u;
+                            const uint32_t hx = ring_load(reinterpret_cast<const uint32_t*>(sb) + 0);
+                            const uint32_t hrow = ring_load(reinterpret_cast<const uint32_t*>(sb) + 1);
+                            const uint32_t hmeta = ring_load(reinterpret_cast<const uint32_t*>(sb) + 2);
+                            const float* r = sb + 3u + g * p.upp * 3u;
+                            float sum_r = 0.f, sum_g = 0.f, sum_b = 0.f;
+                            cstrip = hmeta & 0xffu;
+                            if (!PLAIN && p.s_begin != 0u && g < ((hmeta >> 8) & 0xffu)) {
+                                const float* a = p.strips[cstrip].acc + ((size_t)hrow * p.W + hx + g) * 3;
+                                sum_r = a[0];
+                                sum_g = a[1];
+                                sum_b = a[2];
+                            }
+                            {
+                                uint32_t i = 0;
+                                auto batch = [&](auto cb_tag) {
+                                    constexpr int CB = decltype(cb_tag)::value;
 #pragma clang loop unroll(disable)
-                                for (; i + (uint32_t)CB <= p.upp; i += (uint32_t)CB) {
+                                    for (; i + (uint32_t)CB <= p.upp; i += (uint32_t)CB) {
+                                        LCOUNT(12);
+                                        float c[3 * CB];
+#pragma unroll
+                                        for (int e = 0; e < 3 * CB; e++) c[e] = ring_load(r + e);
+#pragma unroll
+                                        for (int e = 0; e < CB; e++) {
+                                            sum_r = sum_r + c[3 * e + 0];
+                                            sum_g = sum_g + c[3 * e + 1];
+                                            sum_b = sum_b + c[3 * e + 2];
+                                        }
+                                        r += 3 * CB;
+                                    }
+                                };
+                                if (RT_COMMIT_BATCH > 4 && !QNODES) batch(std::integral_constant<int, RT_COMMIT_BATCH>{});
+                                batch(std::integral_constant<int, 4>{});
+#pragma clang loop unroll(disable)
+                                for (; i < p.upp; i++) {
                                     LCOUNT(12);
-                                    float c[3 * CB];
-#pragma unroll
-                                    for (int e = 0; e < 3 * CB; e++) c[e] = ring_load(r + e);
-#pragma unroll
-                                    for (int e = 0; e < CB; e++) {
-                                        sum_r = sum_r + c[3 * e + 0];
-                                        sum_g = sum_g + c[3 * e + 1];
-                                        sum_b = sum_b + c[3 * e + 2];
-                                    }
-                                    r += 3 * CB;
-                                }
-                            };
-                            if (RT_COMMIT_BATCH > 4 && !QNODES) batch(std::integral_constant<int, RT_COMMIT_BATCH>{});
-                            batch(std::integral_constant<int, 4>{});
-#pragma clang loop unroll(disable)
-                            for (; i < p.upp; i++) {
-                                LCOUNT(12);
-                                const float cr = ring_load(r + 0);
-                                const float cg = ring_load(r + 1);
-                                const float cb = ring_load(r + 2);
-                                sum_r = sum_r + cr;
-                                sum_g = sum_g + cg;
-                                sum_b = sum_b + cb;
-                                r += 3;
-                            }
-                        }
-                        if (g < ((hmeta >> 8) & 0xffu)) {
-                            float cr_, cg_, cb_;
-                            if (p.spp_rcp != 0.0f) {
-                                cr_ = __builtin_sqrtf(sum_r * p.spp_rcp);
-                                cg_ = __builtin_sqrtf(sum_g * p.spp_rcp);
-                                cb_ = __builtin_sqrtf(sum_b * p.spp_rcp);
-                            } else {
-                                cr_ = __builtin_sqrtf(sum_r / p.spp_f);
-                                cg_ = __builtin_sqrtf(sum_g / p.spp_f);
-                                cb_ = __builtin_sqrtf(sum_b / p.spp_f);
-                            }
-                            const uint32_t sidx = hmeta & 0xffu;
-                            stg = (hmeta >> 16) & 0xffu;
-                            const size_t oidx = ((size_t)hrow * p.W + hx + g) * 3;
-                            if (p.acc_out) {
-                                float* a = p.strips[sidx].acc;
-                                a[oidx + 0] = sum_r;
-                                a[oidx + 1] = sum_g;
-                                a[oidx + 2] = sum_b;
-                            }
-                            if (!CAN_STAGE || stg == STAGE_TILES) {
-                                uint8_t* orgb = p.strips[sidx].rgb;
-                                orgb[oidx + 0] = f32_as_u8(cr_ * 255.999f);
-                                orgb[oidx + 1] = f32_as_u8(cg_ * 255.999f);
-                                orgb[oidx + 2] = f32_as_u8(cb_ * 255.999f);
-                            } else {
-                                uint8_t* sd = stage_base + stg * STAGE_TILE_BYTES + ((hx + g) & 63u) * 3u;
-                                sd[0] = f32_as_u8(cr_ * 255.999f);
-                                sd[1] = f32_as_u8(cg_ * 255.999f);
-                                sd[2] = f32_as_u8(cb_ * 255.999f);
-                                fin = true;
-                            }
-                            float* of = p.strips[sidx].f32;
-                            if (of) {
-                                of[oidx + 0] = cr_;
-                                of[oidx + 1] = cg_;
-                                of[oidx + 2] = cb_;
-                            }
-                            (void)pin;
-                        }
-                    }
-                    if (p.strip_cost && mine && g == 0u) {
-                        const uint32_t sg = wq.cnt[slot & (SLOTS_MAX - 1u)] >> SLOT_UNIT_BITS;
-                        if (cstrip == wq.cost_strip[0]) (void)__hip_atomic_fetch_add(&wq.cost_acc[0], sg, __ATOMIC_RELAXED, __HIP_MEMORY_SCOPE_WAVEFRONT);
-                        else if (cstrip == wq.cost_strip[1]) (void)__hip_atomic_fetch_add(&wq.cost_acc[1], sg, __ATOMIC_RELAXED, __HIP_MEMORY_SCOPE_WAVEFRONT);
-                        else if (sg) atomicAdd(&p.strip_cost[(blockIdx.x % COST_COPIES) * MAX_BATCH + cstrip], (unsigned long long)sg);
-                    }
-                    if (CAN_STAGE && __ballot(fin)) {
-                        __builtin_amdgcn_fence(__ATOMIC_ACQ_REL, "wavefront");
-#pragma unroll
-                        for (uint32_t k = 0; k < STAGE_TILES; k++) {
-                            const unsigned long long mk = __ballot(fin && stg == k);
-                            if (mk == 0ull) continue;
-                            const int left = (int)uni((uint32_t)wst.left[k]) - (int)__builtin_popcountll(mk);
-                            if (left == 0) {
-                                if (lane < (int)(STAGE_TILE_BYTES / 4)) {
-                                    uint32_t* d32 = reinterpret_cast<uint32_t*>(((uintptr_t)uni(wst.dst_hi[k]) << 32) | uni(wst.dst_lo[k]));
-                                    d32[lane] = reinterpret_cast<const uint32_t*>(stage_base + k * STAGE_TILE_BYTES)[lane];
+                                    const float cr = ring_load(r + 0);
+                                    const float cg = ring_load(r + 1);
+                                    const float cb = ring_load(r + 2);
+                                    sum_r = sum_r + cr;
+                                    sum_g = sum_g + cg;
+                                    sum_b = sum_b + cb;
+                                    r += 3;
                                 }
                             }
-                            if (lane == 0) wst.left[k] = left == 0 ? -1 : left;
-                        }
-                        __builtin_amdgcn_fence(__ATOMIC_ACQ_REL, "wavefront");
-                    }
-                }
+                            if (g < ((hmeta >> 8) & 0xffu)) {
+                                float cr_, cg_, cb_;
+                                if (PLAIN || p.spp_rcp != 0.0f) {
+                                    cr_ = __builtin_sqrtf(sum_r * p.spp_rcp);
+                                    cg_ = __builtin_sqrtf(sum_g * p.spp_rcp);
+                                    cb_ = __builtin_sqrtf(sum_b * p.spp_rcp);
+                                } else {
+                                    cr_ = __builtin_sqrtf(sum_r / p.spp_f);
+                                    cg_ = __builtin_sqrtf(sum_g / p.spp_f);
+                                    cb_ = __builtin_sqrtf(sum_b / p.spp_f);
+                                }
+                                const uint32_t sidx = hmeta & 0xffu;
+                                stg = (hmeta >> 16) & 0xffu;
+                                const size_t oidx = ((size_t)hrow * p.W + hx + g) * 3;
+                                if (!PLAIN && p.acc_out) {
+                                    float* a = p.strips[sidx].acc;
+                                    a[oidx + 0] = sum_r;
+                                    a[oidx + 1] = sum_g;
+                                    a[oidx + 2] = sum_b;
+                                }
+                                if (!CAN_STAGE || stg == STAGE_TILES) {
+                                    uint8_t* orgb = p.strips[sidx].rgb;
+                                    orgb[oidx + 0] = f32_as_u8(cr_ * 255.999f);
+                                    orgb[oidx + 1] = f32_as_u8(cg_ * 255.999f);
+                                    orgb[oidx + 2] = f32_as_u8(cb_ * 255.999f);
+                                } else {
+                                    uint8_t* sd = stage_base + stg * STAGE_TILE_BYTES + ((hx + g) & 63u) * 3u;
+                                    sd[0] = f32_as_u8(cr_ * 255.999f);
+                                    sd[1] = f32_as_u8(cg_ * 255.999f);
+                                    sd[2] = f32_as_u8(cb_ * 255.999f);
+                                    fin = true;
+                                }
+                                float* of = PLAIN ? nullptr : p.strips[sidx].f32;
+                                if (of) {
+                                    of[oidx + 0] = cr_;
+                                    of[oidx + 1] = cg_;
+                                    of[oidx + 2] = cb_;
+                                }
+                                (void)pin;
+                            }
+                        }
+                        if (!PLAIN && p.strip_cost && mine && g == 0u) {
+                            const uint32_t sg = wq.cnt[slot & (SLOTS_MAX - 1u)] >> SLOT_UNIT_BITS;
+                            if (cstrip == wq.cost_strip[0]) (void)__hip_atomic_fetch_add(&wq.cost_acc[0], sg, __ATOMIC_RELAXED, __HIP_MEMORY_SCOPE_WAVEFRONT);
+                            else if (cstrip == wq.cost_strip[1]) (void)__hip_atomic_fetch_add(&wq.cost_acc[1], sg, __ATOMIC_RELAXED, __HIP_MEMORY_SCOPE_WAVEFRONT);
+                            else if (sg) atomicAdd(&p.strip_cost[(blockIdx.x % COST_COPIES) * MAX_BATCH + cstrip], (unsigned long long)sg);
+                        }
+                        if (CAN_STAGE && __ballot(fin)) {
+                            __builtin_amdgcn_fence(__ATOMIC_ACQ_REL, "wavefront");
+#pragma unroll
+                            for (uint32_t k = 0; k < STAGE_TILES; k++) {
+                                const unsigned long long mk = __ballot(fin && stg == k);
+                                if (mk == 0ull) continue;
+                                const int left = (int)uni((uint32_t)wst.left[k]) - (int)__builtin_popcountll(mk);
+                                if (left == 0) {
+                                    if (lane < (int)(STAGE_TILE_BYTES / 4)) {
+                                        uint32_t* d32 = reinterpret_cast<uint32_t*>(((uintptr_t)uni(wst.dst_hi[k]) << 32) | uni(wst.dst_lo[k]));
+                                        d32[lane] = reinterpret_cast<const uint32_t*>(stage_base + k * STAGE_TILE_BYTES)[lane];
+                                    }
+                                }
+                                if (lane == 0) wst.left[k] = left == 0 ? -1 : left;
+                            }
+                            __builtin_amdgcn_fence(__ATOMIC_ACQ_REL, "wavefront");
+                        }
+                    }
+                };
+                if (PLAIN_OK && p.plain != 0u) commit_complete(std::true_type{});
+                else commit_complete(std::false_type{});
                 if (slot_done) wq.cnt[cold<QNODES>(lane)] = SLOT_FREE;
                 freem = uni(freem | complete);
                 __builtin_amdgcn_fence(__ATOMIC_ACQ_REL, "wavefront");
@@ -1022,7 +1031,7 @@
                     const uint32_t prim = p.big[j];
                     float t;
                     bool hit;
-                    if (prim < p.n_sph) {
+                    if (!TRIS || prim < p.n_sph) {
                         const float4 g = RT_SPHERE_REC(p, prim);
                         hit = exact_sphere(o, 2.0f * d, mk(g.x, g.y, g.z), g.w, p.t_min, p.t_max, t);
                     } else {
@@ -1046,7 +1055,7 @@
                     const uint32_t prim = LTREE ? (uint32_t)lc16[i * BLOCK + tid16] & 0x7fffu
                                           : p.list16 ? (uint32_t)lc16[i * BLOCK + tid16] : lc32[i * BLOCK + tid];
                     float t;
-                    if (prim < p.n_sph) {
+                    if (!TRIS || prim < p.n_sph) {
                         const float4 g = RT_SPHERE_REC(p, prim);
                         if (exact_sphere(o, 2.0f * d, mk(g.x, g.y, g.z), g.w, p.t_min, p.t_max, t)) {
                             if (QNODES)
@@ -1615,7 +1624,7 @@
                 m = at32(p.mat, (uint32_t)h.idx);
                 if (!(em > 0.0f)) {
                     hp = o + h.t * d;
-                    if ((uint32_t)h.idx < p.n_sph) {
+                    if (!TRIS || (uint32_t)h.idx < p.n_sph) {
                         float4 g = TRAVERSE ? RT_SPHERE_REC(p, (uint32_t)h.idx) : at32(p.geom, (uint32_t)h.idx);
                         nv = hp - mk(g.x, g.y, g.z);
                     } else {
@@ -1634,7 +1643,7 @@
                     finished = true;
                 } else {
                     const V3 n = nn;
-                    if (p.path32)
+                    if (path32())
                         reinterpret_cast<uint32_t*>(lpath)[k * BLOCK + cold<QNODES>(tid)] = (uint32_t)h.idx;
                     else
                         reinterpret_cast<uint16_t*>(lpath)[k * BLOCK + cold<QNODES>(tid16)] = (uint16_t)h.idx;
@@ -1673,7 +1682,7 @@
                 LCOUNT(10);
                 {
                     auto path_idx = [&](uint32_t i) -> uint32_t {
-                        return p.path32 ? reinterpret_cast<uint32_t*>(lpath)[i * BLOCK + cold<QNODES>(tid)]
+                        return path32() ? reinterpret_cast<uint32_t*>(lpath)[i * BLOCK + cold<QNODES>(tid)]
                                         : (uint32_t) reinterpret_cast<uint16_t*>(lpath)[i * BLOCK + cold<QNODES>(tid16)];
                     };
                     uint32_t i = k;
@@ -1721,7 +1730,7 @@
 
 using KernelFn = void (*)(const KParams);
 KernelFn kernel_linear(int isect, bool expanded);
-KernelFn kernel_traverse(int isect, bool stats);
+KernelFn kernel_traverse(int isect, bool stats, bool tris = true);
 void sqrt_selftest_launch(uint32_t from, unsigned long long n, unsigned long long* d_bad, hipStream_t st);
 
 }
diff --git a/ray_tracer_s8_amd/csrc/rt_kernels_trav.hip b/ray_tracer_s8_amd/csrc/rt_kernels_trav.hip
--- a/ray_tracer_s8_amd/csrc/rt_kernels_trav.hip
+++ b/ray_tracer_s8_amd/csrc/rt_kernels_trav.hip
@@ -2,10 +2,10 @@
 
 namespace rtk {
 template <bool STATS>
-KernelFn traverse_kernel(int isect) {
+KernelFn traverse_kernel(int isect, bool tris) {
     switch (isect) {
-        case 5: return rt_tile_kernel<5, false, LTREE_BLOCK, STATS>;
-        case 6: return rt_tile_kernel<6, false, LTREE_BLOCK, STATS>;
+        case 5: return tris ? rt_tile_kernel<5, false, LTREE_BLOCK, STATS, true> : rt_tile_kernel<5, false, LTREE_BLOCK, STATS, false>;
+        case 6: return tris ? rt_tile_kernel<6, false, LTREE_BLOCK, STATS, true> : rt_tile_kernel<6, false, LTREE_BLOCK, STATS, false>;
         case 7: return rt_tile_kernel<7, false, BLOCK, STATS>;
         case 8: return rt_tile_kernel<8, false, BLOCK, STATS>;
         case 9: return rt_tile_kernel<9, false, BLOCK, STATS>;
@@ -15,7 +15,7 @@
         default: return nullptr;
     }
 }
-KernelFn kernel_traverse(int isect, bool stats) { return stats ? traverse_kernel<true>(isect) : traverse_kernel<false>(isect); }
+KernelFn kernel_traverse(int isect, bool stats, bool tris) { return stats ? traverse_kernel<true>(isect, tris) : traverse_kernel<false>(isect, tris); }
 
 __global__ void sqrt_selftest_kernel(uint32_t from, unsigned long long n, unsigned long long* bad) {
     unsigned long long mine = 0;
diff --git a/ray_tracer_s8_amd/csrc/rt_plan.h b/ray_tracer_s8_amd/csrc/rt_plan.h
--- a/ray_tracer_s8_amd/csrc/rt_plan.h
+++ b/ray_tracer_s8_amd/csrc/rt_plan.h
@@ -49,6 +49,8 @@
     int compact = 1;
     int refill_eighths = 0;
     int tail_tiles = -1;
+    int ltree_general = 0;
+    int plain_frame = 1;
 };
 
 struct Engine {
@@ -80,6 +82,8 @@
     int block = rtk::BLOCK;
     bool expanded = false;
     bool count_steps = false;
+    bool tris = true;
+    bool plain_shape = false;
     size_t lds = 0;
     uint32_t maxl_l2 = 0;
     uint32_t ovf_entries = 0;
@@ -87,6 +91,12 @@
     size_t ring_bytes = 0;
     size_t ovf_words = 0;
 };
+
+constexpr uint32_t LT_MAX_PRIMS = 0x7fffu;
+constexpr uint32_t PATH16_MAX_PRIMS = 65536u;
+constexpr uint32_t LT_SPHERE_ONLY_MAX_TRIS = 0;
+
+inline bool plain_frame(const Plan& pl, bool any_f32, bool strip_cost) { return pl.plain_shape && !any_f32 && !strip_cost; }
 
 inline bool cull_wanted(uint32_t flags, int knob, bool rule) {
     return (flags & RT_FLAG_NO_CULL_WALK) ? false : (flags & RT_FLAG_CULL_WALK) ? true : knob >= 0 ? knob != 0 : rule;
@@ -220,7 +230,8 @@
     const bool traverse = trav_ok && ((fl & RT_FLAG_BVH_TRAVERSE) || (n_prims >= TRAVERSE_MIN_PRIMS && !dense_pile));
     bool ltree_fits = false;
     const size_t lt_lane = ((size_t)MAXL_LTREE + (size_t)(rq.max_bounces + 1) + (size_t)(sh.bvh_depth + 2)) * sizeof(uint16_t);
-    if (traverse && kn.lds_tree != 0 && !(fl & RT_FLAG_NO_LDS_TREE) && sh.n_internal > 0 && n_prims <= 0x7fffu &&
+    static_assert(LT_MAX_PRIMS <= PATH16_MAX_PRIMS, "the LDS-tree kernels compile the 32-bit path entries out (rt_kernel.hip.h path32())");
+    if (traverse && kn.lds_tree != 0 && !(fl & RT_FLAG_NO_LDS_TREE) && sh.n_internal > 0 && n_prims <= LT_MAX_PRIMS &&
         ((size_t)sh.n_internal + 2) * LNODE_DW < 0x8000u) {
         const size_t fixed = (((size_t)sh.n_internal + 2) * LNODE_DW + n_prims) * 4 + 16 + lt_lane * LTREE_BLOCK;
         ltree_fits = fixed <= LDS_LIMIT;
@@ -242,7 +253,7 @@
     const int bs = ENGINES[pl.engine].block;
     p.chunk = traverse ? 0 : (streamed ? STREAM_CHUNK : sh.n_sph_pad);
     p.n_chunks = p.chunk ? (sh.n_sph_pad + p.chunk - 1) / p.chunk : 0;
-    p.path32 = (sh.n_sph + sh.n_tri) > 65536u ? 1u : 0u;
+    p.path32 = (sh.n_sph + sh.n_tri) > PATH16_MAX_PRIMS ? 1u : 0u;
     size_t geom_bytes = traverse ? 0 : (size_t)(p.chunk ? p.chunk : 1) * 4 * sizeof(float);
     p.lds_cand_off = (uint32_t)geom_bytes;
     size_t path_bytes = (size_t)p.depth * BLOCK * (p.path32 ? 4 : 2);
@@ -314,6 +325,7 @@
     pl.block = bs;
     pl.expanded = expanded;
     pl.count_steps = traverse && (fl & RT_FLAG_COUNT_STEPS);
+    pl.tris = !(ltree && sh.n_tri <= LT_SPHERE_ONLY_MAX_TRIS && kn.ltree_general == 0);
     pl.maxl_l2 = maxl;
     pl.ovf_entries = pl.capped ? stack_capped - stack_lds : 0u;
     fill_camera(rq, pose, p);
@@ -349,6 +361,7 @@
     p.tiles_total = (uint32_t)n_tiles;
     p.n_tiles = (uint32_t)n_tiles;
     p.tiles_big = (uint32_t)n_tiles;
+    pl.plain_shape = ltree && kn.plain_frame != 0 && p.s_begin == 0u && p.acc_out == 0u && p.grp == 1u && p.spp_rcp != 0.0f && p.path32 == 0u;
     return pl;
 }
 
```

Result: faster. 16150, median of 6 (+2.1%).
